# jwliao1209/DiffMusic

Measured on AMD Instinct MI355X. Metric: denoising steps/sec (10 s clip, 200-step DPS), higher is better.
Workload: dtype f16; 1 GPU; MusicLDM + DPS music_inpainting, 10 s @16 kHz, 200-step schedule, batch 8 per GPU (BASELINE.json configs[1]); global_batch=8, clips_per_gpu=8, lanes=1, parallelism=clip-sharded x1 (RCCL world size 1, no per-step collective), finite=True, nan_steps=0, settle_steps=10, cached_reference_transform=True, launched_by=single process

## Files before the change

diffmusic_amd/_ctypes_ops.py:

```python
import ctypes as C

import torch

from . import _lib


def _stream():
    return C.c_void_p(torch.cuda.current_stream().cuda_stream)


def _p(t):
    return C.c_void_p(t.data_ptr()) if t is not None else C.c_void_p(0)


def abi_version():
    return _lib.lib().dmx_abi_version()


def sched_pred_x0(x, eps, alpha_t, *, ptype=0, clip_r=0.0):
    x0 = torch.empty_like(x)
    if ptype == 0 and clip_r == 0.0:
        _lib.check(_lib.lib().dmx_sched_pred_x0(_p(x), _p(eps), _p(x0), x.numel(), alpha_t, _stream()), "pred_x0")
    else:
        _lib.check(_lib.lib().dmx_sched_pred_x0_ex(_p(x), _p(eps), _p(x0), x.numel(), alpha_t, ptype, clip_r, _stream()), "pred_x0_ex")
# ... 461 lines not shown
    return mean, logvar, x


def grad_normalize_(dwav, target):
    inv_scale = torch.empty(dwav.shape[0], dtype=torch.float32, device=dwav.device)
    _lib.check(_lib.lib().dmx_grad_normalize(_p(dwav), _p(inv_scale), dwav.shape[0], dwav.shape[1], target, _stream()), "grad_normalize")
    return inv_scale


def hifigan_fwd(model, mel, ws):
    lib = _lib.lib()
    B, T, _ = mel.shape
    wav = torch.empty(B, lib.dmx_hifigan_out_len(model, T), dtype=torch.float32, device=mel.device)
    _lib.check(lib.dmx_hifigan_fwd(model, _p(mel), _p(wav), B, T, _p(ws), ws.numel(), _stream()), "hifigan_fwd")
    return wav


def hifigan_fwd_dead(model, mel, s0, s1, ws):
    B, T, _ = mel.shape
    lib = _lib.lib()
    wav = torch.empty(B, lib.dmx_hifigan_out_len(model, T), dtype=torch.float32, device=mel.device)
    _lib.check(lib.dmx_hifigan_fwd_dead(model, _p(mel), _p(wav), B, T, int(s0), int(s1), _p(ws), ws.numel(), _stream()), "hifigan_fwd_dead")
    return wav


def hifigan_dead_plan(model, stages):
    n = int(stages)
    arr = [(C.c_int * n)() for _ in range(4)]
    if _lib.lib().dmx_hifigan_dead_plan(model, *arr, n) < 0:
        _lib.check(-1, "hifigan_dead_plan")
    return [int(a[s]) for s in range(n) for a in arr]


def hifigan_bwd(model, dwav, frames, model_in_dim):
    dmel = torch.empty(dwav.shape[0], frames, model_in_dim, dtype=_lib.act_dtype(), device=dwav.device)
    _lib.check(_lib.lib().dmx_hifigan_bwd(model, _p(dwav), _p(dmel), _stream()), "hifigan_bwd")
    return dmel


def htsat_fwd(model, mel, keep_state, ws):
    lib = _lib.lib()
    B, frames, _ = mel.shape
    tokens, channels = C.c_int(), C.c_int()
    _lib.check(lib.dmx_htsat_feature_dims(model, C.byref(tokens), C.byref(channels)), "htsat dims")
    feat = torch.empty(B, tokens.value, channels.value, dtype=torch.float32, device=mel.device)
    _lib.check(lib.dmx_htsat_fwd(model, _p(mel), B, frames, _p(feat), int(keep_state), _p(ws), ws.numel(), _stream()), "htsat_fwd")
    return feat


def htsat_bwd(model, dfeat, scale, frames, bins):
    dmel = torch.empty(dfeat.shape[0], frames, bins, dtype=torch.float32, device=dfeat.device)
    _lib.check(_lib.lib().dmx_htsat_bwd(model, _p(dfeat), _p(scale), _p(dmel), _stream()), "htsat_bwd")
    return dmel


def gram_fwd(feat):
    B, T, Cc = feat.shape
    g = torch.empty(B, Cc, Cc, dtype=torch.float32, device=feat.device)
    _lib.check(_lib.lib().dmx_gram_fwd(_p(feat), _p(g), B, T, Cc, _stream()), "gram_fwd")
    return g


def gram_bwd(feat, dgram):
    B, T, Cc = feat.shape
    d = torch.empty_like(feat)
    _lib.check(_lib.lib().dmx_gram_bwd(_p(feat), _p(dgram), _p(d), B, T, Cc, _stream()), "gram_bwd")
# ... 2 lines not shown
```

diffmusic_amd/_lib.py:

```python
import ctypes as C
import os

_HERE = os.path.dirname(os.path.abspath(__file__))
LIB_PATH = os.environ.get("DMX_LIB_PATH") or os.path.join(_HERE, "lib", "libdiffmusic_hip.so")
MAX_STAGES = 8


class HifiGanConfig(C.Structure):
    _fields_ = [("model_in_dim", C.c_int), ("upsample_initial_channel", C.c_int), ("num_upsamples", C.c_int),
                ("upsample_rates", C.c_int * MAX_STAGES), ("upsample_kernel_sizes", C.c_int * MAX_STAGES),
                ("num_kernels", C.c_int), ("resblock_kernel_sizes", C.c_int * MAX_STAGES),
                ("num_dilations", C.c_int), ("resblock_dilation_sizes", C.c_int * (MAX_STAGES * MAX_STAGES)),
                ("leaky_relu_slope", C.c_float)]


class VaeConfig(C.Structure):
    _fields_ = [("latent_channels", C.c_int), ("out_channels", C.c_int), ("num_blocks", C.c_int),
                ("block_out_channels", C.c_int * MAX_STAGES), ("layers_per_block", C.c_int),
                ("norm_num_groups", C.c_int), ("eps", C.c_float)]


class UNetConfig(C.Structure):
    _fields_ = [("in_channels", C.c_int), ("out_channels", C.c_int), ("num_blocks", C.c_int),
                ("block_out_channels", C.c_int * MAX_STAGES), ("layers_per_block", C.c_int),
# ... 26 lines not shown
                ("XB", C.c_void_p), ("B2", C.c_void_p), ("ldxb", C.c_int), ("ldb2", C.c_int),
                ("colsum", C.c_void_p), ("ln_eps", C.c_float), ("rowstats_in", C.c_void_p), ("rowstats_out", C.c_void_p), ("nslots", C.c_int),
                ("gn_part", C.c_void_p), ("gnb_x", C.c_void_p), ("gnb_scale", C.c_void_p), ("gnb_shift", C.c_void_p),
                ("gnb_ldx", C.c_int), ("gnb_silu", C.c_int), ("gnb_stats", C.c_void_p), ("gnb_cpg", C.c_int)]


EPI_BIAS, EPI_ROWBIAS, EPI_RESID, EPI_ACCUM, EPI_MASK, EPI_LRELU2, EPI_TANH, EPI_F32OUT, EPI_NO_C, EPI_RESID_INV, EPI_MASKBITS, EPI_BITS2, EPI_SOFTBWD = \
    1, 2, 4, 8, 16, 32, 64, 128, 256, 512, 1024, 2048, 4096
EPI_GEGLU, EPI_LNFOLD, EPI_ROWSTATS, EPI_GNSTATS, EPI_GNBWD = 8192, 16384, 32768, 65536, 131072

_SIGS = {
    "dmx_abi_version": (C.c_int, []),
    "dmx_act_dtype": (C.c_int, []),
    "dmx_last_error": (C.c_char_p, []),
    "dmx_hifigan_create": (C.c_void_p, [C.POINTER(HifiGanConfig)]),
    "dmx_vae_decoder_create": (C.c_void_p, [C.POINTER(VaeConfig)]),
    "dmx_unet_create": (C.c_void_p, [C.POINTER(UNetConfig)]),
    "dmx_model_destroy": (None, [C.c_void_p]),
    "dmx_model_num_params": (C.c_int, [C.c_void_p]),
    "dmx_model_param_name": (C.c_char_p, [C.c_void_p, C.c_int]),
    "dmx_model_param_numel": (C.c_size_t, [C.c_void_p, C.c_int]),
    "dmx_model_param_ndim": (C.c_int, [C.c_void_p, C.c_int]),
    "dmx_model_param_dim": (C.c_int, [C.c_void_p, C.c_int, C.c_int]),
    "dmx_model_load_param": (C.c_int, [C.c_void_p, C.c_char_p, C.c_void_p, C.c_size_t]),
    "dmx_model_finalize": (C.c_int, [C.c_void_p, C.c_void_p]),
    "dmx_hifigan_out_len": (C.c_int, [C.c_void_p, C.c_int]),
    "dmx_hifigan_workspace_bytes": (C.c_size_t, [C.c_void_p, C.c_int, C.c_int]),
    "dmx_hifigan_fwd": (C.c_int, [C.c_void_p, C.c_void_p, C.c_void_p, C.c_int, C.c_int, C.c_void_p, C.c_size_t, C.c_void_p]),
    "dmx_hifigan_bwd": (C.c_int, [C.c_void_p, C.c_void_p, C.c_void_p, C.c_void_p]),
    "dmx_hifigan_fwd_dead": (C.c_int, [C.c_void_p, C.c_void_p, C.c_void_p, C.c_int, C.c_int, C.c_int, C.c_int, C.c_void_p, C.c_size_t,
                                       C.c_void_p]),
    "dmx_hifigan_dead_plan": (C.c_int, [C.c_void_p, C.POINTER(C.c_int), C.POINTER(C.c_int), C.POINTER(C.c_int), C.POINTER(C.c_int), C.c_int]),
    "dmx_conv_dead_rows": (C.c_int, [C.c_int] * 9 + [C.POINTER(C.c_int), C.POINTER(C.c_int)]),
    "dmx_vae_workspace_bytes": (C.c_size_t, [C.c_void_p, C.c_int, C.c_int, C.c_int]),
    "dmx_vae_decode_fwd": (C.c_int, [C.c_void_p, C.c_void_p, C.c_float, C.c_void_p, C.c_void_p, C.c_int, C.c_int, C.c_int,
                                     C.c_int, C.c_void_p, C.c_size_t, C.c_void_p]),
    "dmx_vae_decode_bwd": (C.c_int, [C.c_void_p, C.c_void_p, C.c_float, C.c_void_p, C.c_void_p]),
    "dmx_vae_encoder_create": (C.c_void_p, [C.POINTER(VaeConfig)]),
    "dmx_vae_encoder_workspace_bytes": (C.c_size_t, [C.c_void_p, C.c_int, C.c_int, C.c_int]),
    "dmx_vae_encode_fwd": (C.c_int, [C.c_void_p, C.c_void_p, C.c_float, C.c_void_p, C.c_int, C.c_int, C.c_int, C.c_void_p, C.c_size_t,
                                     C.c_void_p]),
    "dmx_latent_init": (C.c_int, [C.c_void_p] * 6 + [C.c_int] * 3 + [C.c_float] * 3 + [C.c_void_p]),
    "dmx_conv2d_raw": (C.c_int, [C.c_void_p] * 4 + [C.c_int] * 9 + [C.c_void_p]),
    "dmx_unet_workspace_bytes": (C.c_size_t, [C.c_void_p, C.c_int, C.c_int, C.c_int]),
    "dmx_unet_fwd": (C.c_int, [C.c_void_p, C.c_void_p, C.c_void_p, C.c_void_p, C.c_void_p, C.c_int, C.c_int, C.c_int,
                               C.c_void_p, C.c_size_t, C.c_void_p]),
    "dmx_unet_fwd_ctx": (C.c_int, [C.c_void_p] * 5 + [C.c_int, C.c_void_p, C.c_int, C.c_void_p, C.c_void_p, C.c_int, C.c_int, C.c_int,
                                   C.c_void_p, C.c_size_t, C.c_void_p]),
    "dmx_unet_workspace_bytes_ctx": (C.c_size_t, [C.c_void_p, C.c_int, C.c_int, C.c_int, C.c_int, C.c_int]),
    "dmx_htsat_create": (C.c_void_p, [C.POINTER(HtsatConfig)]),
    "dmx_htsat_feature_dims": (C.c_int, [C.c_void_p, C.POINTER(C.c_int), C.POINTER(C.c_int)]),
    "dmx_htsat_workspace_bytes": (C.c_size_t, [C.c_void_p, C.c_int, C.c_int]),
    "dmx_htsat_fwd": (C.c_int, [C.c_void_p, C.c_void_p, C.c_int, C.c_int, C.c_void_p, C.c_int, C.c_void_p, C.c_size_t, C.c_void_p]),
    "dmx_htsat_bwd": (C.c_int, [C.c_void_p, C.c_void_p, C.c_void_p, C.c_void_p, C.c_void_p]),
    "dmx_htsat_tape_raw": (C.c_size_t, [C.c_void_p, C.c_int, C.c_int, C.c_int, C.c_void_p, C.c_size_t, C.c_void_p]),
    "dmx_gram_fwd": (C.c_int, [C.c_void_p, C.c_void_p, C.c_int, C.c_int, C.c_int, C.c_void_p]),
    "dmx_gram_bwd": (C.c_int, [C.c_void_p, C.c_void_p, C.c_void_p, C.c_int, C.c_int, C.c_int, C.c_void_p]),
    "dmx_gemm_raw": (C.c_int, [C.c_void_p, C.c_size_t, C.c_void_p]),
    "dmx_prof_begin": (None, []),
    "dmx_prof_end": (C.c_int, [C.POINTER(C.c_double), C.POINTER(C.c_double)]),
    "dmx_flash_attn_raw": (C.c_int, [C.c_void_p, C.c_void_p, C.c_void_p, C.c_void_p, C.c_void_p] + [C.c_int] * 6 + [C.c_float, C.c_void_p]),
    "dmx_flash_attn_ld_raw": (C.c_int, [C.c_void_p] * 5 + [C.c_int] * 8 + [C.c_float, C.POINTER(C.c_int), C.c_void_p]),
    "dmx_softmax_raw": (C.c_int, [C.c_void_p] * 3 + [C.c_longlong, C.c_int, C.c_longlong, C.c_longlong, C.c_int, C.c_void_p]),
    "dmx_softmax_act_raw": (C.c_int, [C.c_void_p] * 3 + [C.c_longlong, C.c_int, C.c_longlong, C.c_int, C.c_void_p]),
    "dmx_transpose_raw": (C.c_int, [C.c_void_p, C.c_void_p, C.c_int, C.c_int, C.c_longlong, C.c_longlong, C.c_int, C.c_int] + [C.c_longlong] * 4
                          + [C.c_void_p]),
# ... 58 lines not shown
                                     C.c_void_p]),
    "dmx_audio_tf_wgrad_segments": (C.c_int, [C.c_int]),
    "dmx_audio_tf_wgrad": (C.c_int, [C.c_void_p, C.c_void_p, C.c_longlong, C.c_void_p, C.c_longlong, C.c_void_p, C.c_int, C.c_int, C.c_void_p]),
    "dmx_audio_eq_update": (C.c_int, [C.c_void_p, C.c_int] + [C.c_void_p] * 3 + [C.c_int, C.c_int] + [C.c_double] * 4 + [C.c_int, C.c_void_p]),
    "dmx_audio_melscale": (C.c_int, [C.c_void_p, C.c_void_p, C.c_void_p, C.c_int, C.c_int, C.c_float, C.c_float, C.c_void_p]),
    "dmx_mask_apply": (C.c_int, [C.c_void_p, C.c_longlong, C.c_void_p, C.c_void_p, C.c_longlong, C.c_int, C.c_int, C.c_int, C.c_void_p]),
    "dmx_l2_loss": (C.c_int, [C.c_void_p, C.c_longlong, C.c_void_p, C.c_void_p, C.c_void_p, C.c_int, C.c_longlong, C.c_float, C.c_void_p]),
    "dmx_track_stitch_fwd": (C.c_int, [C.c_void_p, C.c_longlong, C.c_void_p, C.POINTER(C.c_int)] + [C.c_int] * 4 + [C.c_void_p]),
    "dmx_track_stitch_bwd": (C.c_int, [C.c_void_p, C.c_void_p, C.c_longlong, C.POINTER(C.c_int)] + [C.c_int] * 5 + [C.c_void_p]),
    "dmx_stem_mix_fwd": (C.c_int, [C.c_void_p, C.c_longlong, C.c_void_p, C.POINTER(C.c_float)] + [C.c_int] * 3 + [C.c_void_p]),
    "dmx_stem_mix_bwd": (C.c_int, [C.c_void_p, C.c_void_p, C.c_longlong, C.POINTER(C.c_float)] + [C.c_int] * 4 + [C.c_void_p]),
    "dmx_stem_project": (C.c_int, [C.c_void_p, C.c_longlong, C.c_void_p, C.c_void_p, C.POINTER(C.c_float), C.c_int, C.c_int, C.c_void_p]),
    "dmx_grad_normalize": (C.c_int, [C.c_void_p, C.c_void_p, C.c_int, C.c_longlong, C.c_float, C.c_void_p]),
    "dmx_fir_fwd": (C.c_int, [C.c_void_p, C.c_longlong, C.c_void_p, C.c_void_p, C.c_longlong] + [C.c_int] * 7 + [C.c_void_p]),
    "dmx_fir_bwd": (C.c_int, [C.c_void_p, C.c_longlong, C.c_void_p, C.c_void_p, C.c_void_p, C.c_longlong] + [C.c_int] * 7 + [C.c_void_p]),
    "dmx_fir_clip_fwd": (C.c_int, [C.c_void_p, C.c_longlong, C.c_void_p, C.c_void_p, C.c_longlong] + [C.c_int] * 4 + [C.c_void_p]),
    "dmx_fir_clip_bwd": (C.c_int, [C.c_void_p, C.c_longlong, C.c_void_p, C.c_void_p, C.c_void_p, C.c_longlong] + [C.c_int] * 4 + [C.c_void_p]),
    "dmx_fir_wgrad_workspace_floats": (C.c_size_t, [C.c_int, C.c_int, C.c_int]),
    "dmx_fir_wgrad": (C.c_int, [C.c_void_p, C.c_longlong, C.c_void_p, C.c_longlong, C.c_void_p, C.c_size_t] + [C.c_int] * 4 + [C.c_void_p]),
    "dmx_ir_update": (C.c_int, [C.c_void_p, C.c_int] + [C.c_void_p] * 4 + [C.c_int, C.c_int] + [C.c_double] * 4 + [C.c_int, C.c_void_p]),
    "dmx_sched_pred_x0": (C.c_int, [C.c_void_p, C.c_void_p, C.c_void_p, C.c_longlong, C.c_float, C.c_void_p]),
    "dmx_sched_pred_x0_ex": (C.c_int, [C.c_void_p, C.c_void_p, C.c_void_p, C.c_longlong, C.c_float, C.c_int, C.c_float, C.c_void_p]),
    "dmx_sched_step_ex": (C.c_int, [C.c_int] + [C.c_void_p] * 9 + [C.c_int, C.c_int] + [C.c_float] * 5 + [C.c_int, C.c_int, C.c_float, C.c_void_p]),
    "dmx_sched_cfg_combine": (C.c_int, [C.c_void_p, C.c_void_p, C.c_longlong, C.c_float, C.c_void_p]),
    "dmx_randn_philox": (C.c_int, [C.c_void_p, C.c_int, C.c_longlong, C.POINTER(C.c_ulonglong), C.c_ulonglong, C.c_void_p]),
    "dmx_sched_step": (C.c_int, [C.c_int] + [C.c_void_p] * 9 + [C.c_int, C.c_int] + [C.c_float] * 5 + [C.c_int, C.c_void_p]),
}

ADDED_IN_V4 = ("dmx_vae_encoder_create", "dmx_vae_encoder_workspace_bytes", "dmx_vae_encode_fwd", "dmx_latent_init",
               "dmx_track_stitch_fwd", "dmx_track_stitch_bwd", "dmx_audio_guidance_fwd_shaped", "dmx_audio_guidance_bwd_shaped",
               "dmx_clip_fwd", "dmx_clip_bwd", "dmx_declip_project", "dmx_hifigan_fwd_dead", "dmx_hifigan_dead_plan", "dmx_conv_dead_rows",
               "dmx_fir_clip_fwd", "dmx_fir_clip_bwd", "dmx_fir_wgrad", "dmx_fir_wgrad_workspace_floats", "dmx_ir_update",
               "dmx_stem_mix_fwd", "dmx_stem_mix_bwd", "dmx_stem_project", "dmx_audio_tf_gain", "dmx_audio_tf_frames",
               "dmx_audio_tf_curve", "dmx_audio_tf_wgrad_segments", "dmx_audio_tf_wgrad", "dmx_audio_eq_update", "dmx_drc_fwd", "dmx_drc_bwd")

_lib = None


def check_symbols(h, path=LIB_PATH):
    for name in ADDED_IN_V4:
        if not hasattr(h, name):
            raise RuntimeError(f"{path} reports ABI version {ABI_VERSION} but does not export `{name}` (a build from before the VAE "
                               "encoder / track-mode / declipping / blind-dereverberation / source-separation / time-frequency-masking / blind-equalisation / de-compression entry points): rebuild it (python -m diffmusic_amd.build --force)")


def lib():
    global _lib
    if _lib is None:
        if not os.path.exists(LIB_PATH):
            raise RuntimeError(f"{LIB_PATH} is missing: build it with `python -m diffmusic_amd.build` "
                               "(the diffmusic_amd hot path has no CPU fallback)")
        h = C.CDLL(LIB_PATH)
        for name, (res, args) in _SIGS.items():
            if not hasattr(h, name):
                continue
            fn = getattr(h, name)
            fn.restype, fn.argtypes = res, args
        if h.dmx_abi_version() != ABI_VERSION:
            raise RuntimeError(f"libdiffmusic_hip.so ABI version {h.dmx_abi_version()} != {ABI_VERSION} expected by this package: rebuild it "
                               "(python -m diffmusic_amd.build --force)")
        check_symbols(h)
        _lib = h
    return _lib


ABI_VERSION = 4


def act_dtype():
    import torch
    return torch.float16 if lib().dmx_act_dtype() == 1 else torch.bfloat16


class DmxError(RuntimeError):
    pass

# ... 6 lines not shown
```

diffmusic_amd/csrc/capi.hip:

```cpp
#include "conv_pair.h"
#include "models.h"

#define M_IMPL(m) ((m) ? (m)->impl : nullptr)
#define ST(s) ((hipStream_t)(s))

extern "C" {

int dmx_abi_version(void) { return DMX_ABI_VERSION; }
int dmx_act_dtype(void) { return DMX_ACT_DTYPE; }

dmx_model* dmx_hifigan_create(const dmx_hifigan_config* cfg) {
  if (!cfg || cfg->num_upsamples > DMX_MAX_STAGES || cfg->num_kernels > DMX_MAX_STAGES || cfg->num_dilations > DMX_MAX_STAGES) {
    dmx_set_error("bad hifigan config");
    return nullptr;
  }
  return new dmx_model{dmx_make_hifigan(cfg)};
}
dmx_model* dmx_vae_decoder_create(const dmx_vae_config* cfg) {
  if (!cfg || cfg->num_blocks > DMX_MAX_STAGES) { dmx_set_error("bad vae config"); return nullptr; }
  Model* m = dmx_make_vae(cfg);
  return m ? new dmx_model{m} : nullptr;
}
dmx_model* dmx_unet_create(const dmx_unet_config* cfg) {
  if (!cfg || cfg->num_blocks > DMX_MAX_STAGES) { dmx_set_error("bad unet config"); return nullptr; }
// ... 16 lines not shown
}
int dmx_model_finalize(dmx_model* m, void* stream) {
  std::string missing;
  if (!m->impl->ps.all_loaded(&missing)) { dmx_set_error("parameter '%s' was never loaded", missing.c_str()); return DMX_ERR_PARAM; }
  const int rc = m->impl->finalize(ST(stream));
  if (rc == DMX_OK) m->impl->finalized = true;
  return rc;
}

static int check(dmx_model* m, int kind) {
  if (!m || !m->impl || m->impl->kind != kind) { dmx_set_error("wrong model handle"); return DMX_ERR_STATE; }
  if (!m->impl->finalized) { dmx_set_error("model not finalized"); return DMX_ERR_STATE; }
  return DMX_OK;
}

int dmx_hifigan_out_len(const dmx_model* m, int frames) { return dmx_hifigan_out_len_impl(m->impl, frames); }
size_t dmx_hifigan_workspace_bytes(dmx_model* m, int batch, int frames) { return dmx_hifigan_ws_impl(m->impl, batch, frames); }
int dmx_hifigan_fwd(dmx_model* m, const uint16_t* mel, float* wav, int batch, int frames, void* ws, size_t ws_bytes, void* stream) {
  int rc = check(m, DMX_MODEL_HIFIGAN);
  if (rc) return rc;
  if (!ws) { dmx_set_error("null workspace"); return DMX_ERR_WORKSPACE; }
  return dmx_hifigan_fwd_impl(m->impl, mel, wav, batch, frames, ws, ws_bytes, ST(stream));
}
int dmx_hifigan_fwd_dead(dmx_model* m, const uint16_t* mel, float* wav, int batch, int frames, int s0, int s1, void* ws, size_t ws_bytes,
                         void* stream) {
  int rc = check(m, DMX_MODEL_HIFIGAN);
  if (rc) return rc;
  if (!ws || !mel || !wav) { dmx_set_error("hifigan_fwd_dead: null buffer"); return DMX_ERR_STATE; }
  return dmx_hifigan_fwd_dead_impl(m->impl, mel, wav, batch, frames, s0, s1, ws, ws_bytes, ST(stream));
}
int dmx_hifigan_dead_plan(dmx_model* m, int* skipped, int* total, int* lo, int* hi, int n) {
  if (!m || !m->impl || m->impl->kind != DMX_MODEL_HIFIGAN) { dmx_set_error("wrong model handle"); return -1; }
  return dmx_hifigan_dead_plan_impl(m->impl, skipped, total, lo, hi, n);
}
int dmx_conv_dead_rows(int k, int dil, int pad, int stride, int transposed, int t_in, int t_out, int a, int b, int* lo, int* hi) {
  if (!lo || !hi) return DMX_ERR_STATE;
  return dmx_conv_dead_rows_impl(k, dil, pad, stride, transposed, t_in, t_out, a, b, lo, hi);
}
int dmx_hifigan_bwd(dmx_model* m, const float* dwav, uint16_t* dmel, void* stream) {
  int rc = check(m, DMX_MODEL_HIFIGAN);
  if (rc) return rc;
  return dmx_hifigan_bwd_impl(m->impl, dwav, dmel, ST(stream));
}

size_t dmx_vae_workspace_bytes(dmx_model* m, int batch, int h, int w) { return dmx_vae_ws_impl(m->impl, batch, h, w); }
int dmx_vae_decode_fwd(dmx_model* m, const float* z, float z_scale, uint16_t* mel, float* mel_f32, int batch, int h, int w,
                       int keep_state, void* ws, size_t ws_bytes, void* stream) {
  int rc = check(m, DMX_MODEL_VAE);
  if (rc) return rc;
  if (!ws) { dmx_set_error("null workspace"); return DMX_ERR_WORKSPACE; }
  return dmx_vae_fwd_impl(m->impl, z, z_scale, mel, mel_f32, batch, h, w, keep_state, ws, ws_bytes, ST(stream));
}
int dmx_vae_decode_bwd(dmx_model* m, const uint16_t* dmel, float z_scale, float* dz, void* stream) {
  int rc = check(m, DMX_MODEL_VAE);
  if (rc) return rc;
  return dmx_vae_bwd_impl(m->impl, dmel, z_scale, dz, ST(stream));
}

dmx_model* dmx_vae_encoder_create(const dmx_vae_config* cfg) {
  if (!cfg || cfg->num_blocks > DMX_MAX_STAGES) { dmx_set_error("bad vae config"); return nullptr; }
  Model* m = dmx_make_vae_encoder(cfg);
  return m ? new dmx_model{m} : nullptr;
}
size_t dmx_vae_encoder_workspace_bytes(dmx_model* m, int batch, int frames, int bins) {
  if (!m || !m->impl || m->impl->kind != DMX_MODEL_VAE_ENC) return 0;
  return dmx_vae_enc_ws_impl(m->impl, batch, frames, bins);
// ... 240 lines not shown
```

diffmusic_amd/csrc/dmx_common.h:

```cpp
#pragma once
#include <hip/hip_runtime.h>
#include <stdint.h>
#include <stddef.h>

typedef uint16_t act_t;

#define DMX_OK 0
#define DMX_ERR_SHAPE (-1)
#define DMX_ERR_WORKSPACE (-2)
#define DMX_ERR_PARAM (-3)
#define DMX_ERR_STATE (-4)
#define DMX_ERR_LAUNCH (-5)

typedef __attribute__((ext_vector_type(4))) float f32x4;
#ifdef DMX_BF16
typedef __bf16 native16_t;
typedef __attribute__((ext_vector_type(8))) __bf16 frag8_t;
#define DMX_MFMA16(a, b, c) __builtin_amdgcn_mfma_f32_16x16x32_bf16(a, b, c, 0, 0, 0)
#define DMX_ACT_DTYPE 0
#else
typedef _Float16 native16_t;
typedef __attribute__((ext_vector_type(8))) _Float16 frag8_t;
#define DMX_MFMA16(a, b, c) __builtin_amdgcn_mfma_f32_16x16x32_f16(a, b, c, 0, 0, 0)
#define DMX_ACT_DTYPE 1
// ... 83 lines not shown
  int M, N, K;
  int ldw;
  int Hi, Wi, Ci, lda;
  int Hq, Wq, sy, sx;
  int ntaps;
  int Ho, Wo, ldc, osy, ooy, osx, oox;
  int ldr, ldx, ldc2;
  int Z, Zi;
  long long sAo, sAi, sWo, sWi, sCo, sCi;
  float alpha, act_slope, mask_slope;
  int flags;
  signed char tdy[DMX_MAX_TAPS], tdx[DMX_MAX_TAPS];
  float resid_inv_slope;
  int tile_cfg;
  int ldrb;
  int ksplit;
  const unsigned char* XB;
  unsigned char* B2;
  int ldxb, ldb2;
  const float* colsum;
  float ln_eps;
  const float* rowstats_in;
  float* rowstats_out;
  int nslots;
  float* gn_part;
  const act_t* gnb_x;
  const float* gnb_scale;
  const float* gnb_shift;
  int gnb_ldx, gnb_silu;
  const float* gnb_stats;
  int gnb_cpg;
};

int dmx_gemm_launch(const GemmDesc& d, hipStream_t stream, int* gn_rows = nullptr);
void dmx_gemm_set_splitk_workspace(float* ws, size_t bytes);
void dmx_gemm_release_splitk_workspace(const float* ws);
int dmx_gemm_launch_ln(int cfg, const GemmDesc& d, hipStream_t stream);
int dmx_gemm_launch_rowstats(int cfg, const GemmDesc& d, hipStream_t stream);
int dmx_gemm_launch_gnstats(int cfg, const GemmDesc& d, hipStream_t stream, int* gn_rows);
bool dmx_prof_is_active();
```

diffmusic_amd/csrc/gemm_conv.hip:

```cpp
#include "gemm_tile.h"

namespace {
template <int BM, int BN, int WM, int WN, int NSTAGE>
int launch_glds(const GemmDesc& d, hipStream_t stream) {
  if (d.flags & EPI_SOFTBWD) {
    if constexpr (BM == 256 && BN == 256) return launch_glds_t<BM, BN, WM, WN, NSTAGE, 2>(d, stream);
    else return DMX_ERR_SHAPE;
  }
  if (d.flags & EPI_GEGLU) return launch_glds_t<BM, BN, WM, WN, NSTAGE, 3>(d, stream);
  return (d.flags & (EPI_MASKBITS | EPI_BITS2)) ? launch_glds_t<BM, BN, WM, WN, NSTAGE, 1>(d, stream)
                                                : launch_glds_t<BM, BN, WM, WN, NSTAGE, 0>(d, stream);
}

template <int BM, int BN, int WM, int WN>
int launch_cfg(const GemmDesc& d, hipStream_t stream) {
  if (d.flags & EPI_SOFTBWD) return DMX_ERR_SHAPE;
  if (d.flags & EPI_GEGLU) {
    if constexpr ((BN / WN) % 32 == 0) return launch_cfg_t<BM, BN, WM, WN, 3>(d, stream);
    else return DMX_ERR_SHAPE;
  }
  return (d.flags & (EPI_MASKBITS | EPI_BITS2)) ? launch_cfg_t<BM, BN, WM, WN, 1>(d, stream) : launch_cfg_t<BM, BN, WM, WN, 0>(d, stream);
}

}

#include <vector>
#include <cstdio>
#include <cstdlib>
#include <cmath>
namespace {
struct ProfRec { hipEvent_t a, b; double flops, bytes; int M, N, K, Z, taps, flags, cfg; };
int g_last_cfg = 0;
bool g_prof = false;
std::vector<ProfRec> g_prof_recs;
struct TileEntry { int M, N, K, Z, cfg; };
static const TileEntry g_tile_table[] = {
#include "tile_table.inc"
    {0, 0, 0, 0, 0}};

bool glds_ok(const GemmDesc& d) {
  const long long imgs = d.Hq * d.Wq > 0 ? (d.M + (long long)d.Hq * d.Wq - 1) / ((long long)d.Hq * d.Wq) : 1;
  const long long in_elems = (d.Hi > 1 || d.ntaps > 1 ? imgs * d.Hi * d.Wi : (long long)d.M) * d.lda;
  static const bool strided_ok = getenv("DMX_NO_GLDS_STRIDED") == nullptr;
  return in_elems < (1ll << 29) && (long long)d.M * d.lda < (1ll << 29) && ((long long)d.N + 512) * d.ldw < (1ll << 29) &&
         (d.sy == 1 || strided_ok);
}
int launch_by_cfg(int cfg, const GemmDesc& d, hipStream_t stream, int* gn_rows = nullptr) {
  g_last_cfg = cfg;
  if (d.flags & EPI_LNFOLD) return dmx_gemm_launch_ln(cfg, d, stream);
  if (d.flags & EPI_ROWSTATS) return dmx_gemm_launch_rowstats(cfg, d, stream);
  if (d.flags & (EPI_GNSTATS | EPI_GNBWD)) return dmx_gemm_launch_gnstats(cfg, d, stream, gn_rows);
  switch (cfg) {
    case 1: return launch_glds<256, 256, 2, 4, 2>(d, stream);
    case 2: return launch_glds<256, 128, 4, 2, 3>(d, stream);
    case 7: return launch_glds<320, 256, 2, 4, 2>(d, stream);
    case 8: return launch_glds<192, 256, 2, 4, 2>(d, stream);
    case 9: return launch_glds<320, 128, 4, 2, 2>(d, stream);
    case 10: return launch_glds<192, 128, 4, 2, 3>(d, stream);
    case 11: return launch_glds<128, 128, 2, 2, 2>(d, stream);
    case 12: return launch_glds<64, 64, 2, 2, 4>(d, stream);
    case 13: return launch_glds<128, 64, 2, 2, 3>(d, stream);
    case 14: return launch_glds<64, 128, 2, 2, 3>(d, stream);
    case 15: return launch_glds<64, 64, 2, 2, 8>(d, stream);
    case 16: return launch_glds<64, 128, 2, 2, 6>(d, stream);
    case 17: return launch_glds<128, 64, 2, 2, 6>(d, stream);
    case 18: return launch_glds<128, 128, 2, 2, 4>(d, stream);
    case 19: return launch_glds<512, 128, 4, 2, 2>(d, stream);
    case 3: return launch_cfg<128, 128, 2, 2>(d, stream);
    case 4: return launch_cfg<128, 64, 2, 2>(d, stream);
    case 5: return launch_cfg<128, 32, 4, 1>(d, stream);
    default: return launch_cfg<64, 64, 2, 2>(d, stream);
  }
}
int launch_dispatch(const GemmDesc& d, hipStream_t stream, int* gn_rows) {
  const bool gl = glds_ok(d);
  if (d.flags & EPI_SOFTBWD) return gl ? launch_by_cfg(1, d, stream, gn_rows) : DMX_ERR_SHAPE;
  if (d.tile_cfg >= 1 && d.tile_cfg <= 19 && ((d.tile_cfg > 2 && d.tile_cfg < 7) || gl)) return launch_by_cfg(d.tile_cfg, d, stream, gn_rows);
  {
    static int ovN[8], ovC[8], nov = -1;
    if (nov < 0) {
      nov = 0;
      if (const char* e = getenv("DMX_CFG_OVERRIDE")) {
        while (*e && nov < 8) {
          int n = 0, c = 0;
          if (sscanf(e, "%d:%d", &n, &c) == 2) { ovN[nov] = n; ovC[nov] = c; ++nov; }
          while (*e && *e != ',') ++e;
          if (*e == ',') ++e;
        }
      }
    }
    if (gl && d.M >= 40000)
      for (int i = 0; i < nov; ++i) if (ovN[i] == d.N) return launch_by_cfg(ovC[i], d, stream, gn_rows);
  }
  for (const TileEntry* e = g_tile_table; e->cfg; ++e)
    if (e->M == d.M && e->N == d.N && e->K == d.K && e->Z == d.Z) {
      const int c = e->cfg % 100;
      if ((c > 2 && c < 7) || gl) return launch_by_cfg(c, d, stream, gn_rows);
    }
  if (gl && d.M >= 2048 && d.N % 128 == 0) {
    auto cost = [&](int bm, int bn, int slots, double eff) {
      const double blocks = (double)cdiv(d.M, bm) * cdiv(d.N, bn) * d.Z;
      const double rounds = ceil(blocks / slots);
      return rounds * (bm / 128.0) * (bn / 128.0) * (slots / 256.0) / eff;
    };
    struct Cand { int cfg, bm, bn, slots; double eff; };
    static const Cand cands[] = {{1, 256, 256, 256, 0.95}, {7, 320, 256, 256, 0.93}, {8, 192, 256, 256, 0.88},
                                 {2, 256, 128, 256, 0.70}, {9, 320, 128, 256, 0.70}, {10, 192, 128, 256, 0.66},
                                 {19, 512, 128, 256, 0.75},
                                 {3, 128, 128, 512, 0.66}};
    int best = 0;
    double bc = 1e30;
    for (const Cand& c : cands) {
      if (c.bn == 256 && d.N % 256) continue;
      const double v = cost(c.bm, c.bn, c.slots, c.eff);
      if (v < bc) { bc = v; best = c.cfg; }
    }
    if (best && best != 3) return launch_by_cfg(best, d, stream, gn_rows);
  }
  if (d.N > 32 && (long long)cdiv(d.M, 128) * cdiv(d.N, 128) * d.Z < 200) {
    if (gl && d.K >= 512 && d.Z == 1) return launch_by_cfg(d.N % 128 == 0 && d.M >= 4000 ? 14 : 12, d, stream, gn_rows);
    return launch_by_cfg(6, d, stream, gn_rows);
  }
  if (d.N > 64) return launch_by_cfg(3, d, stream, gn_rows);
  if (d.N > 32) return launch_by_cfg(4, d, stream, gn_rows);
  return launch_by_cfg(5, d, stream, gn_rows);
}
}

bool dmx_prof_is_active() { return g_prof; }

extern "C" void dmx_prof_begin(void) {
  for (auto& r : g_prof_recs) { (void)hipEventDestroy(r.a); (void)hipEventDestroy(r.b); }
  g_prof_recs.clear();
  g_prof = true;
}
static double g_dma_ms = 0.0, g_dma_fl = 0.0, g_dma_by = 0.0;
static int g_dma_n = 0;
#ifdef DMX_GEMM_STAMPS
extern "C" int dmx_gemm_stamps_read(unsigned long long* host) {
  return hipMemcpyFromSymbol(host, HIP_SYMBOL(g_gemm_stamps), sizeof(unsigned long long) * 8192 * 6) == hipSuccess ? 0 : -1;
}
#endif

extern "C" int dmx_prof_dominant(double* ms, double* flops, double* bytes) {
  if (ms) *ms = g_dma_ms;
  if (flops) *flops = g_dma_fl;
  if (bytes) *bytes = g_dma_by;
  return g_dma_n;
}
extern "C" int dmx_prof_end(double* total_ms, double* total_flops) {
  g_prof = false;
  g_dma_ms = g_dma_fl = g_dma_by = 0.0; g_dma_n = 0;
  (void)hipDeviceSynchronize();
  double ms = 0.0, fl = 0.0;
  FILE* csv = getenv("DMX_PROF_CSV") ? fopen(getenv("DMX_PROF_CSV"), "w") : nullptr;
  if (csv) fprintf(csv, "M,N,K,Z,taps,flags,cfg,ms,tflops\n");
  for (auto& r : g_prof_recs) {
    float t = 0.f;
    if (hipEventElapsedTime(&t, r.a, r.b) == hipSuccess) ms += t;
    if (csv) fprintf(csv, "%d,%d,%d,%d,%d,%d,%d,%.4f,%.1f\n", r.M, r.N, r.K, r.Z, r.taps, r.flags, r.cfg, t, t > 0 ? r.flops / t / 1e9 : 0.0);
    const bool dma = r.cfg == 1 || r.cfg == 2 || (r.cfg >= 7 && r.cfg <= 10) || r.cfg == 19;
    if (dma) { g_dma_ms += t; g_dma_fl += r.flops; g_dma_by += r.bytes; ++g_dma_n; }
    fl += r.flops;
    (void)hipEventDestroy(r.a); (void)hipEventDestroy(r.b);
  }
  if (csv) fclose(csv);
  const int n = (int)g_prof_recs.size();
  g_prof_recs.clear();
  if (total_ms) *total_ms = ms;
  if (total_flops) *total_flops = fl;
  return n;
}

namespace {
float* g_splitk_ws = nullptr;
size_t g_splitk_bytes = 0;

__global__ void splitk_epilogue_kernel(const GemmDesc p, const float* __restrict__ ws, int ksplit) {
  const long long q = (long long)blockIdx.x * blockDim.x + threadIdx.x;
  const int nq = p.N >> 2;
  if (q >= (long long)p.M * nq) return;
  const int m = (int)(q / nq), n = (int)(q - (long long)m * nq) * 4;
  const long long mn = (long long)p.M * p.N;
  float4 v = *reinterpret_cast<const float4*>(ws + (long long)m * p.N + n);
  for (int s = 1; s < ksplit; ++s) {
    const float4 w = *reinterpret_cast<const float4*>(ws + s * mn + (long long)m * p.N + n);
    v.x += w.x; v.y += w.y; v.z += w.z; v.w += w.w;
  }
  float a[4] = {v.x, v.y, v.z, v.w};
  const int flags = p.flags;
  const long long row = m;
  if (flags & EPI_MASK) {
    const uint2 xr = *reinterpret_cast<const uint2*>(p.X + row * p.ldx + n);
    const float x[4] = {alo(xr.x), ahi(xr.x), alo(xr.y), ahi(xr.y)};
// ... 60 lines not shown
  g.flags = EPI_F32OUT;
  g.C = g_splitk_ws; g.C2 = nullptr; g.ldc = d.N; g.alpha = 1.f;
  g.bias = nullptr; g.rowbias = nullptr; g.R = nullptr; g.X = nullptr;
  g.Ho = d.Hq; g.Wo = d.Wq;
  g.tile_cfg = 0;
  int rc = launch_by_cfg(tile, g, stream);
  if (rc != DMX_OK) return rc;
  const long long nthr = (long long)d.M * (d.N >> 2);
  hipLaunchKernelGGL(splitk_epilogue_kernel, dim3((unsigned)((nthr + 255) / 256)), dim3(256), 0, stream, d, g_splitk_ws, ks);
  g_last_cfg = 100 * ks + tile;
  return hipGetLastError() == hipSuccess ? DMX_OK : DMX_ERR_LAUNCH;
}
}

void dmx_gemm_set_splitk_workspace(float* ws, size_t bytes) { g_splitk_ws = ws; g_splitk_bytes = bytes; }
void dmx_gemm_release_splitk_workspace(const float* ws) { if (g_splitk_ws == ws) { g_splitk_ws = nullptr; g_splitk_bytes = 0; } }

int dmx_prof_open(hipStream_t st) {
  if (!g_prof) return -1;
  ProfRec r;
  memset(&r, 0, sizeof(r));
  (void)hipEventCreate(&r.a); (void)hipEventCreate(&r.b);
  (void)hipEventRecord(r.a, st);
  g_prof_recs.push_back(r);
  return (int)g_prof_recs.size() - 1;
}
void dmx_prof_close(int rec, hipStream_t st, double flops, double bytes, int M, int N, int K, int taps, int flags, int cfg) {
  if (rec < 0 || rec >= (int)g_prof_recs.size()) return;
  ProfRec& r = g_prof_recs[rec];
  (void)hipEventRecord(r.b, st);
  r.flops = flops; r.bytes = bytes; r.M = M; r.N = N; r.K = K; r.Z = 1; r.taps = taps; r.flags = flags; r.cfg = cfg;
}

int dmx_gemm_launch(const GemmDesc& d, hipStream_t stream, int* gn_rows) {
  if (gn_rows) *gn_rows = 0;
  if (d.M <= 0 || d.N <= 0 || d.K <= 0) return DMX_ERR_SHAPE;
  if ((d.Ci & 7) || (d.N & 3) || (d.K & 7) || (d.lda & 7) || (d.ldw & 7) || (d.ldc & 3)) return DMX_ERR_SHAPE;
  if (d.ntaps < 1 || d.ntaps > DMX_MAX_TAPS || d.K != d.ntaps * d.Ci) return DMX_ERR_SHAPE;
  if (d.Z < 1 || d.Zi < 1) return DMX_ERR_SHAPE;
  if ((d.flags & EPI_LRELU2) && !(d.act_slope >= 0.f && d.act_slope <= 1.f)) return DMX_ERR_SHAPE;
  if ((d.flags & EPI_RESID_INV) && !(d.resid_inv_slope >= 1.f)) return DMX_ERR_SHAPE;
  if (d.flags & EPI_SOFTBWD) {
    if ((d.flags & ~(EPI_SOFTBWD)) || ((d.N | d.ldc | d.ldx) & 7) || !d.X || !d.rowbias || d.Zi != 1 || d.ntaps != 1) return DMX_ERR_SHAPE;
    if (!(d.osy == 1 && d.osx == 1 && d.ooy == 0 && d.oox == 0 && d.Ho == d.Hq && d.Wo == d.Wq)) return DMX_ERR_SHAPE;
  }
  if (d.flags & EPI_GEGLU) {
    if ((d.flags & ~(EPI_GEGLU | EPI_BIAS | EPI_LNFOLD)) || (d.N & 31) || (d.ldc & 7) || d.ldc < d.N / 2 || d.alpha != 1.f) return DMX_ERR_SHAPE;
    if ((d.ldr | d.ldx | d.ldc2) & 7) return DMX_ERR_SHAPE;
    if (!(d.osy == 1 && d.osx == 1 && d.ooy == 0 && d.oox == 0 && d.Ho == d.Hq && d.Wo == d.Wq)) return DMX_ERR_SHAPE;
  }
  if (d.flags & (EPI_MASKBITS | EPI_BITS2)) {
    if ((d.flags & EPI_F32OUT) || ((d.N | d.ldc | d.ldr | d.ldx | d.ldc2) & 7) || d.Z != 1) return DMX_ERR_SHAPE;
    if ((d.flags & EPI_MASKBITS) && (!d.XB || d.ldxb * 8 < d.N)) return DMX_ERR_SHAPE;
    if ((d.flags & EPI_BITS2) && (!d.B2 || d.ldb2 * 8 < d.N)) return DMX_ERR_SHAPE;
  }
  if ((d.flags & EPI_LNFOLD) && (d.flags & EPI_BIAS)) {
    GemmDesc q = d;
    q.flags &= ~EPI_BIAS;
    return dmx_gemm_launch(q, stream, gn_rows);
  }
  if (d.flags & EPI_LNFOLD) {
    if (d.ntaps != 1 || d.K != d.Ci || !d.colsum || !d.rowstats_in || d.nslots < 1 || d.Z != 1 ||
        (d.flags & (EPI_F32OUT | EPI_MASK | EPI_MASKBITS | EPI_BITS2 | EPI_SOFTBWD | EPI_ACCUM | EPI_TANH | EPI_LRELU2 | EPI_ROWSTATS)))
      return DMX_ERR_SHAPE;
  }
  if (d.flags & EPI_ROWSTATS) {
// ... 40 lines not shown
```

diffmusic_amd/csrc/gemm_epilogue.h:

```cpp
#pragma once
#include "dmx_common.h"
#include <type_traits>

namespace {

template <int I, int N, typename F>
__device__ __forceinline__ void static_for(F&& f) {
  if constexpr (I < N) {
    f(std::integral_constant<int, I>{});
    static_for<I + 1, N>(f);
  }
}


template <int FM, int FN>
__device__ __forceinline__ void gemm_epilogue(const GemmDesc& p, f32x4 (&acc)[FM][FN], int m0, int n0, int lr, int lq,
                                              long long coff, int HqWq) {
  const int flags = p.flags;
#pragma unroll
  for (int i = 0; i < FM; ++i) {
    const int m = m0 + i * 16 + lr;
    if (m >= p.M) continue;
    const int b = m / HqWq, rem = m - b * HqWq;
    const int qy = rem / p.Wq, qx = rem - qy * p.Wq;
// ... 42 lines not shown
        act_t* cp = reinterpret_cast<act_t*>(p.C) + coff + orow * p.ldc + n;
        if (flags & EPI_ACCUM) {
          const uint2 o = *reinterpret_cast<const uint2*>(cp);
          v[0] += alo(o.x); v[1] += ahi(o.x); v[2] += alo(o.y); v[3] += ahi(o.y);
        }
        if (flags & EPI_TANH) { v[0] = tanhf(v[0]); v[1] = tanhf(v[1]); v[2] = tanhf(v[2]); v[3] = tanhf(v[3]); }
        if (!(flags & EPI_NO_C)) *reinterpret_cast<uint2*>(cp) = make_uint2(pack2a(v[0], v[1]), pack2a(v[2], v[3]));
      }
      if (flags & EPI_LRELU2) {
        const float s = p.act_slope;
        const float a0 = v[0] > 0.f ? v[0] : v[0] * s, a1 = v[1] > 0.f ? v[1] : v[1] * s;
        const float a2 = v[2] > 0.f ? v[2] : v[2] * s, a3 = v[3] > 0.f ? v[3] : v[3] * s;
        *reinterpret_cast<uint2*>(p.C2 + coff + orow * p.ldc2 + n) = make_uint2(pack2a(a0, a1), pack2a(a2, a3));
      }
    }
  }
}

__device__ __forceinline__ unsigned dmx_pos8(const uint4& v) {
  auto pos = [](uint32_t u) -> uint32_t { return (((u & 0x7fff7fffu) + 0x7fff7fffu) & ~u) & 0x80008000u; };
  const uint32_t w = (pos(v.x) >> 15) | (pos(v.y) >> 13) | (pos(v.z) >> 11) | (pos(v.w) >> 9);
  return (w & 0x55u) | ((w >> 15) & 0xaau);
}

#ifndef DMX_GNB_HB
#define DMX_GNB_HB 4
#endif
#ifndef DMX_EPI_IB
#define DMX_EPI_IB 4
#endif
template <int FM>
struct EpiChunk { static constexpr int IB = (FM % DMX_EPI_IB == 0) ? DMX_EPI_IB : (FM % 4 == 0) ? 4 : (FM % 3 == 0) ? 3 : (FM % 2 == 0) ? 2 : 1; static constexpr int CH = IB * 16; };

template <int FM, int FN, int EM>
__device__ __forceinline__ void gemm_epilogue_lds_impl(const GemmDesc& p, f32x4 (&acc)[FM][FN], int m0, int n0, int lane,
                                                       long long coff, int HqWq, char* wl, int mlimit,
                                                       const uint2 (&rpre)[FM * FN], const bool use_rpre) {
  constexpr bool BITS = EM == 1;
  constexpr bool SOFT = EM == 2;
  constexpr bool GEGLU = EM == 3;
  constexpr bool ROWS = EM == 4;
  static_assert(!ROWS || FN == 2 || FN == 4, "row statistics come in slots of 32 columns");
  constexpr bool GNS = EM == 5;
  constexpr bool GNB = EM == 6;
  static_assert(!GEGLU || FN % 2 == 0, "GEGLU pairs accumulator fragments");
  constexpr int CH = EpiChunk<FM>::CH;
  constexpr int IB = EpiChunk<FM>::IB;
  constexpr int TNB = FN * 32;
  constexpr int PITCH = TNB + 16;
  constexpr int CPR = TNB / 16;
  constexpr int RPI = 64 / CPR;
  constexpr int NIT = CH / RPI;
  static_assert(CH % RPI == 0, "chunk rows must be a multiple of the rows per wave-instruction");
  const int lr = lane & 15, lq = lane >> 4;
  const int rr = lane / CPR, cch = lane - rr * CPR;
  int* tab = reinterpret_cast<int*>(wl + CH * PITCH);
  const int flags = p.flags;
  const int ncol = n0 + cch * 8;
  const bool col_ok = ncol < p.N;
  const int mend = p.M < mlimit ? p.M : mlimit;
  const bool ident = p.osy == 1 && p.osx == 1 && p.ooy == 0 && p.oox == 0 && p.Ho == p.Hq && p.Wo == p.Wq;
#define DMX_LDS_SYNC() asm volatile("s_waitcnt lgkmcnt(0)" ::: "memory")
  float4 bcol[FN];
#pragma unroll
  for (int j = 0; j < FN; ++j) {
    const int n = n0 + j * 16 + lq * 4;
    bcol[j] = ((flags & EPI_BIAS) && n < p.N) ? *reinterpret_cast<const float4*>(p.bias + n) : make_float4(0.f, 0.f, 0.f, 0.f);
  }
  float gs[4] = {0.f, 0.f, 0.f, 0.f};
  constexpr int GN_SLOT = 64;
  static_assert(!(GNS || GNB) || (CH == GN_SLOT && FN == 4), "GroupNorm statistics: 64-row chunks of 64-column wave tiles only (one summation order)");
  const int gn_b0 = (GNS || GNB) ? m0 / HqWq : 0;
  static_for<0, FM / IB>([&](auto H) {
    constexpr int h = decltype(H)::value;
    int orows[NIT];
    if (ident) {
#pragma unroll
      for (int it = 0; it < NIT; ++it) {
        const int m = m0 + h * CH + it * RPI + rr;
        orows[it] = m < mend ? m : -1;
      }
    } else {
      if (lane < CH) {
        const int m = m0 + h * CH + lane;
        int orow = -1;
        if (m < mend) {
          const int b = m / HqWq, rem = m - b * HqWq;
          const int qy = rem / p.Wq, qx = rem - qy * p.Wq;
          orow = (b * p.Ho + (qy * p.osy + p.ooy)) * p.Wo + (qx * p.osx + p.oox);
        }
        tab[lane] = orow;
      }
      DMX_LDS_SYNC();
#pragma unroll
      for (int it = 0; it < NIT; ++it) orows[it] = tab[it * RPI + rr];
      DMX_LDS_SYNC();
    }
    auto stage_in = [&](const act_t* G, int ld, auto&& f) {
      {
        uint4 v[NIT];
#pragma unroll
        for (int it = 0; it < NIT; ++it) {
          const bool ok = orows[it] >= 0 && col_ok;
          const long long off = ok ? (long long)orows[it] * ld + ncol : 0ll;
          v[it] = *reinterpret_cast<const uint4*>(G + coff + off);
          if (!ok) v[it] = make_uint4(0, 0, 0, 0);
        }
#pragma unroll
        for (int it = 0; it < NIT; ++it) *reinterpret_cast<uint4*>(wl + (it * RPI + rr) * PITCH + cch * 16) = v[it];
      }
      DMX_LDS_SYNC();
#pragma unroll
      for (int ii = 0; ii < IB; ++ii)
#pragma unroll
        for (int j = 0; j < FN; ++j) {
          const uint2 q = *reinterpret_cast<const uint2*>(wl + (ii * 16 + lr) * PITCH + (j * 16 + lq * 4) * 2);
          f(acc[h * IB + ii][j], alo(q.x), ahi(q.x), alo(q.y), ahi(q.y));
        }
      DMX_LDS_SYNC();
    };
    auto stage_out = [&](act_t* G, int ld, auto&& f) {
      constexpr int JS = GEGLU ? 2 : 1;
      static_for<0, IB>([&](auto II) {
        static_for<0, FN / JS>([&](auto JJ) {
          constexpr int ii = decltype(II)::value, j = decltype(JJ)::value * JS;
          float o[4];
          f(acc[h * IB + ii][j], o);
          *reinterpret_cast<uint2*>(wl + (ii * 16 + lr) * PITCH + ((j / JS) * 16 + lq * 4) * 2) = make_uint2(pack2a(o[0], o[1]), pack2a(o[2], o[3]));
        });
      });
      DMX_LDS_SYNC();
      constexpr int HN = NIT > 4 ? NIT / 2 : NIT;
#pragma unroll
      for (int g0 = 0; g0 < NIT; g0 += HN) {
      uint4 v[HN];
#pragma unroll
// ... 175 lines not shown
          if (flags & EPI_ROWBIAS) {
            const float4 bb = *reinterpret_cast<const float4*>(p.rowbias + (long long)bimg * (p.ldrb ? p.ldrb : p.N) + n);
            a[0] += bb.x; a[1] += bb.y; a[2] += bb.z; a[3] += bb.w;
          }
        }
      }
    }
    if constexpr (GEGLU) {
#pragma unroll
      for (int ii = 0; ii < IB; ++ii)
#pragma unroll
        for (int j = 0; j < FN; j += 2) {
          f32x4& a = acc[h * IB + ii][j];
          const f32x4& g = acc[h * IB + ii][j + 1];
#pragma unroll
          for (int e = 0; e < 4; ++e) a[e] *= 0.5f * g[e] * erfcf(g[e] * -0.70710678118654752f);
        }
    }
    if ((flags & EPI_RESID) && use_rpre) {
      const float is = (flags & EPI_RESID_INV) ? p.resid_inv_slope : 1.f;
#pragma unroll
      for (int ii = 0; ii < IB; ++ii)
#pragma unroll
        for (int j = 0; j < FN; ++j) {
          const uint2 q = rpre[(h * IB + ii) * FN + j];
          const float x0 = alo(q.x), x1 = ahi(q.x), x2 = alo(q.y), x3 = ahi(q.y);
          f32x4& a = acc[h * IB + ii][j];
          a[0] += fminf(x0, x0 * is); a[1] += fminf(x1, x1 * is); a[2] += fminf(x2, x2 * is); a[3] += fminf(x3, x3 * is);
        }
    } else if (flags & EPI_RESID) {
      const float is = (flags & EPI_RESID_INV) ? p.resid_inv_slope : 1.f;
      stage_in(p.R, p.ldr, [&](f32x4& a, float x0, float x1, float x2, float x3) {
        a[0] += fminf(x0, x0 * is); a[1] += fminf(x1, x1 * is); a[2] += fminf(x2, x2 * is); a[3] += fminf(x3, x3 * is);
      });
    }
    if (p.alpha != 1.f) {
      const float al = p.alpha;
#pragma unroll
      for (int ii = 0; ii < IB; ++ii)
#pragma unroll
        for (int j = 0; j < FN; ++j) { f32x4& a = acc[h * IB + ii][j]; a[0] *= al; a[1] *= al; a[2] *= al; a[3] *= al; }
    }
    if (flags & EPI_ACCUM)
      stage_in(reinterpret_cast<const act_t*>(p.C), p.ldc, [&](f32x4& a, float x0, float x1, float x2, float x3) { a[0] += x0; a[1] += x1; a[2] += x2; a[3] += x3; });
    if (flags & EPI_TANH) {
#pragma unroll
      for (int ii = 0; ii < IB; ++ii)
#pragma unroll
        for (int j = 0; j < FN; ++j) { f32x4& a = acc[h * IB + ii][j]; a[0] = tanhf(a[0]); a[1] = tanhf(a[1]); a[2] = tanhf(a[2]); a[3] = tanhf(a[3]); }
    }
    if constexpr (ROWS) {
      if (flags & EPI_ROWSTATS) {
        float2* rso = reinterpret_cast<float2*>(p.rowstats_out);
        const int ns = p.nslots;
#pragma unroll
        for (int ii = 0; ii < IB; ++ii) {
          const int m = m0 + h * CH + ii * 16 + lr;
#pragma unroll
          for (int sl = 0; sl < FN / 2; ++sl) {
            float sv = 0.f, qv = 0.f;
#pragma unroll
            for (int jj = 0; jj < 2; ++jj) {
              const int j = sl * 2 + jj;
              const f32x4& a = acc[h * IB + ii][j];
              if (n0 + j * 16 + lq * 4 < p.N) {
                sv += (a[0] + a[1]) + (a[2] + a[3]);
                qv += (a[0] * a[0] + a[1] * a[1]) + (a[2] * a[2] + a[3] * a[3]);
// ... 12 lines not shown
      stage_out(reinterpret_cast<act_t*>(p.C), p.ldc, [&](const f32x4& a, float (&o)[4]) { o[0] = a[0]; o[1] = a[1]; o[2] = a[2]; o[3] = a[3]; });
      if constexpr (BITS) { if (bits2 && !(flags & EPI_LRELU2)) emit_bits(); }
      if constexpr (GNS) { if (flags & EPI_GNSTATS) emit_gn(); }
      if constexpr (GNB) { if (flags & EPI_GNBWD) emit_gnb(); }
      if constexpr (GNS || GNB) {
        if ((flags & (EPI_GNSTATS | EPI_GNBWD)) && m0 + h * CH < mend) {
#pragma unroll
          for (int o = CPR; o < 64; o <<= 1) {
#pragma unroll
            for (int k = 0; k < 4; ++k) gs[k] += __shfl_xor(gs[k], o, 64);
          }
          if (rr == 0 && col_ok) {
            const int nq = p.N >> 2, slots = (HqWq + GN_SLOT - 1) / GN_SLOT + 1;
            float* dst = p.gn_part + (((long long)gn_b0 * slots + (m0 + h * CH - gn_b0 * HqWq) / GN_SLOT) * nq + (ncol >> 2)) * 2;
            *reinterpret_cast<float4*>(dst) = make_float4(gs[0], gs[1], gs[2], gs[3]);
          }
        }
        gs[0] = gs[1] = gs[2] = gs[3] = 0.f;
      }
      DMX_LDS_SYNC();
    }
    if (flags & EPI_LRELU2) {
      const float sl = p.act_slope;
      stage_out(p.C2, p.ldc2, [&](const f32x4& a, float (&o)[4]) {
        o[0] = fmaxf(a[0], a[0] * sl); o[1] = fmaxf(a[1], a[1] * sl); o[2] = fmaxf(a[2], a[2] * sl); o[3] = fmaxf(a[3], a[3] * sl);
      });
      if constexpr (BITS) { if (bits2) emit_bits(); }
      DMX_LDS_SYNC();
    }
  });
#undef DMX_LDS_SYNC
}

template <int FM, int FN, int EM>
__device__ __forceinline__ void gemm_epilogue_lds(const GemmDesc& p, f32x4 (&acc)[FM][FN], int m0, int n0, int lane,
                                                  long long coff, int HqWq, char* wl, int mlimit = 0x7fffffff) {
  const uint2 none[FM * FN] = {};
  gemm_epilogue_lds_impl<FM, FN, EM>(p, acc, m0, n0, lane, coff, HqWq, wl, mlimit, none, false);
}

}
```

diffmusic_amd/csrc/gemm_tile.h:

```cpp
#pragma once
#include "dmx_common.h"
#include <type_traits>
#include <cstdlib>

#include "gemm_epilogue.h"
#include "conv_pair.h"

namespace {

constexpr int BK = 64;
constexpr int DMX_DEF_BIG = 0;

template <int BM, int BN, int NT>
__device__ __forceinline__ void ln_prologue(const GemmDesc& p, int m0, int n0, float2* s_ln, float* s_cs) {
  constexpr int TPR = NT / BM >= 4 ? 4 : (NT / BM >= 2 ? 2 : 1);
  const int tid = threadIdx.x, ns = p.nslots;
  const int r = tid / TPR, sub = tid - r * TPR;
  const float inv_c = 1.f / (float)p.K;
  if (r < BM) {
    const int m = m0 + r;
    const bool row_ok = m < p.M;
    const float2* rs = reinterpret_cast<const float2*>(p.rowstats_in) + (long long)(row_ok ? m : 0) * ns;
    float si = 0.f, qi = 0.f;
    for (int t0 = 0; t0 < ns; t0 += TPR * 8) {
// ... 176 lines not shown
      for (int i = 0; i < FM; ++i) af[i] = *reinterpret_cast<const frag8_t*>(sa + i * 16 * 128 + sw);
#pragma unroll
      for (int j = 0; j < FN; ++j) wf[j] = *reinterpret_cast<const frag8_t*>(sb + j * 16 * 128 + sw);
#pragma unroll
      for (int i = 0; i < FM; ++i)
#pragma unroll
        for (int j = 0; j < FN; ++j)
          acc[i][j] = DMX_MFMA16(wf[j], af[i], acc[i][j]);
    }
    if (ks + 1 < nk) store_tile(cur ^ 1);
    __syncthreads();
  }
  if constexpr (LNF) ln_apply<FM, FN, BN>(acc, s_ln, s_cs, wm * TM, wn * TN, lr, lq);

  if ((p.flags & EPI_F32OUT) || ((p.N | p.ldc | p.ldr | p.ldx | p.ldc2) & 7)) {
    gemm_epilogue<FM, FN>(p, acc, m0t + wm * TM, tn * BN + wn * TN, lr, lq, coff, HqWq);
  } else {
    constexpr int EPI_CH = EpiChunk<FM>::CH;
    constexpr int EPI_WAVE_BYTES = EPI_CH * (FN * 32 + 16) + EPI_CH * 12;
    static_assert(EPI_WAVE_BYTES * WM * WN <= 2 * (BM + BN) * 128, "epilogue staging does not fit the stage buffers");
    gemm_epilogue_lds<FM, FN, EM>(p, acc, m0t + wm * TM, tn * BN + wn * TN, lane, coff, HqWq, smem + wave * EPI_WAVE_BYTES, mlim);
  }
}

constexpr unsigned OOB = 0x80000000u;

#ifdef DMX_GEMM_STAMPS
__device__ unsigned long long g_gemm_stamps[8192 * 6];
#define DMX_GSTAMP(i) do { gstamp_v[i] = wall_clock64(); } while (0)
#else
#define DMX_GSTAMP(i) do { } while (0)
#endif

template <int BM, int BN, int WM, int WN, int NSTAGE, int EM, bool LNF = false>
__device__ __forceinline__ void glds_tile(const GemmDesc& p, char* smem, const int m0, const int tn, const int mlim) {
  constexpr int NW = WM * WN;
  constexpr int TM = BM / WM, TN = BN / WN;
  constexpr int FM = TM / 16, FN = TN / 16;
  constexpr int A_ISS = BM / 8 / NW, B_ISS = BN / 8 / NW;
  constexpr int A_BYTES = BM * 128, B_BYTES = BN * 128, STAGE = A_BYTES + B_BYTES;
  static_assert(A_ISS >= 1 && B_ISS >= 1, "tile too small");

  constexpr int PER = A_ISS + B_ISS;
  constexpr int KEEP = (NSTAGE - 2) * PER;

  const int tid = threadIdx.x;
  const int wave = __builtin_amdgcn_readfirstlane(tid >> 6), lane = tid & 63;
#ifdef DMX_GEMM_STAMPS
  unsigned long long gstamp_v[5] = {0, 0, 0, 0, 0};
#endif
  DMX_GSTAMP(0);
  const int z = blockIdx.y;
  const int zo = z / p.Zi, zi = z - zo * p.Zi;
  const act_t* Ab = p.A + zo * p.sAo + zi * p.sAi;
  const act_t* Wb = p.W + zo * p.sWo + zi * p.sWi;
  const int nsplit = p.ksplit > 1 ? p.ksplit : 1, sp = blockIdx.z;
  const long long coff = zo * p.sCo + zi * p.sCi + (nsplit > 1 ? (long long)sp * p.M * p.N : 0ll);
  const __amdgpu_buffer_rsrc_t rsA = __builtin_amdgcn_make_buffer_rsrc(const_cast<act_t*>(Ab), 0, OOB, 0x00020000);
  const __amdgpu_buffer_rsrc_t rsW = __builtin_amdgcn_make_buffer_rsrc(const_cast<act_t*>(Wb), 0, (unsigned)p.N * (unsigned)p.ldw * 2u, 0x00020000);

  int tapreg = 0;
#pragma unroll
  for (int j = 0; j < DMX_MAX_TAPS; ++j)
    if (lane == j) tapreg = (int)(unsigned char)p.tdy[j] | ((int)(unsigned char)p.tdx[j] << 8);

  const int lrow = lane >> 3, cc = (lane & 7) ^ lrow;
  const int cpt = p.Ci >> 3;
  const int HqWq = p.Hq * p.Wq;
  const unsigned lda2 = (unsigned)p.lda * 2u;
  unsigned a_lin[A_ISS], a_mask2[(A_ISS + 1) / 2];
  {
    int r_iy[A_ISS], r_ix[A_ISS];
    unsigned r_mask[A_ISS];
#pragma unroll
    for (int i = 0; i < A_ISS; ++i) {
      const int m = m0 + (i * NW + wave) * 8 + lrow;
      r_mask[i] = 0u; a_lin[i] = 0u;
      r_iy[i] = -(1 << 20); r_ix[i] = 0;
      if (m < mlim) {
        int b = 0, qy = 0, qx = m;
        if (!(p.Hq == 1 && p.Wq >= p.M)) {
          b = m / HqWq; const int rem = m - b * HqWq;
          qy = rem / p.Wq; qx = rem - qy * p.Wq;
        }
        r_iy[i] = qy * p.sy; r_ix[i] = qx * p.sx;
        a_lin[i] = (unsigned)b * (unsigned)(p.Hi * p.Wi) * lda2 + (unsigned)(r_iy[i] * p.Wi + r_ix[i]) * lda2 + ((unsigned)cc << 4);
      }
    }
    for (int t = 0; t < p.ntaps; ++t) {
      const int tv = __builtin_amdgcn_readlane(tapreg, t);
      const int dy = (int)(signed char)(tv & 0xff), dx = (int)(signed char)((tv >> 8) & 0xff);
#pragma unroll
      for (int i = 0; i < A_ISS; ++i)
        if ((unsigned)(r_iy[i] + dy) < (unsigned)p.Hi && (unsigned)(r_ix[i] + dx) < (unsigned)p.Wi) r_mask[i] |= 1u << t;
    }
#pragma unroll
    for (int i = 0; i < (A_ISS + 1) / 2; ++i) a_mask2[i] = 0u;
#pragma unroll
    for (int i = 0; i < A_ISS; ++i) a_mask2[i >> 1] |= r_mask[i] << ((i & 1) * 16);
  }
  const unsigned ldw2 = (unsigned)p.ldw * 2u;
  const unsigned w_row = (unsigned)(tn * BN + wave * 8 + lrow) * ldw2;
  const unsigned w_step = (unsigned)(NW * 8) * ldw2;

  const int kchunks = p.K >> 3;
  const bool tap_inner = (p.Ci & 63) == 0 || p.ntaps == 1;
  const int cgroups = (p.Ci + 63) >> 6;
  const int nk_all = (p.K + BK - 1) / BK;
  const int ks_per = (nk_all + nsplit - 1) / nsplit;
  const int ks0 = sp * ks_per, ks1 = ks0 + ks_per < nk_all ? ks0 + ks_per : nk_all;
  int i_cg = ks0 / p.ntaps, i_tp = ks0 - i_cg * p.ntaps;
  bool q_kval = false;
  int q_tp = 0;
  unsigned q_adel = 0, q_wdel = 0;
  char* q_base = nullptr;
  auto issue_begin = [&](int ksl, int stage) {
    q_base = smem + stage * STAGE;
    if (tap_inner) {
      const int tp = __builtin_amdgcn_readfirstlane(i_tp), cgi = __builtin_amdgcn_readfirstlane(i_cg);
      q_kval = cgi < cgroups && ksl + ks0 < ks1 && cgi * 8 + cc < cpt;
      const int tv = __builtin_amdgcn_readlane(tapreg, tp);
      const int dy = (int)(signed char)(tv & 0xff), dx = (int)(signed char)((tv >> 8) & 0xff);
      q_tp = tp;
      q_adel = (unsigned)((dy * p.Wi + dx) * (int)lda2) + ((unsigned)cgi << 7);
      q_wdel = (unsigned)(tp * cpt + cgi * 8 + cc) << 4;
      if (++i_tp == p.ntaps) { i_tp = 0; ++i_cg; }
    } else {
// ... 138 lines not shown
        });
      } else {
        static_for<0, NS>([&](auto ST) {
          constexpr int st = decltype(ST)::value;
          read_step(ST);
          wait_step(ST);
          mfma_step(ST);
          if constexpr (st < SPREAD) {
            static_for<st * PER / SPREAD, (st + 1) * PER / SPREAD>(issue_one);
            __builtin_amdgcn_sched_barrier(0);
          }
        });
      }
      asm volatile("s_waitcnt vmcnt(%0)\n\ts_waitcnt lgkmcnt(0)" ::"n"(KEEP) : "memory");
      __builtin_amdgcn_s_barrier();
      cur = cur + 1 == NSTAGE ? 0 : cur + 1;
      nxt = nxt + 1 == NSTAGE ? 0 : nxt + 1;
    }
    if constexpr (LAG) {
      __builtin_amdgcn_sched_barrier(0);
      if (nk > 0) static_for<LOWN, NS>(mfma_step);
    }
  };
  if constexpr (STAGGER) {
    if (wave >= NW / 2) kloop(std::true_type{}); else kloop(std::false_type{});
  } else {
    kloop(std::false_type{});
  }
#undef DMX_DSR
  asm volatile("s_waitcnt vmcnt(0)" ::: "memory");
  __builtin_amdgcn_s_barrier();
  DMX_GSTAMP(2);
  if constexpr (LNF) ln_apply<FM, FN, BN>(acc, s_ln, s_cs, wm * TM, wn * TN, lr, lq);
  if ((p.flags & EPI_F32OUT) || ((p.N | p.ldc | p.ldr | p.ldx | p.ldc2) & 7)) {
    gemm_epilogue<FM, FN>(p, acc, m0 + wm * TM, tn * BN + wn * TN, lr, lq, coff, HqWq);
  } else {
    constexpr int EPI_CH = EpiChunk<FM>::CH;
    constexpr int EPI_WAVE_BYTES = EPI_CH * (FN * 32 + 16) + EPI_CH * 12;
    static_assert(EPI_WAVE_BYTES * WM * WN <= 2 * (BM + BN) * 128, "epilogue staging does not fit the stage buffers");
    gemm_epilogue_lds<FM, FN, EM>(p, acc, m0 + wm * TM, tn * BN + wn * TN, lane, coff, HqWq, smem + wave * EPI_WAVE_BYTES, mlim);
  }
#ifdef DMX_GEMM_STAMPS
  DMX_GSTAMP(3);
  asm volatile("s_waitcnt vmcnt(0)" ::: "memory");
  DMX_GSTAMP(4);
  {
    const int wg = blockIdx.x + gridDim.x * (blockIdx.y + gridDim.y * blockIdx.z);
    if (tid == NW * 64 - 64 && wg < 8192) {
      unsigned hw, xcc;
      asm volatile("s_getreg_b32 %0, hwreg(HW_REG_HW_ID)" : "=s"(hw));
      asm volatile("s_getreg_b32 %0, hwreg(HW_REG_XCC_ID)" : "=s"(xcc));
#pragma unroll
      for (int i = 0; i < 5; ++i) g_gemm_stamps[wg * 6 + i] = gstamp_v[i];
      g_gemm_stamps[wg * 6 + 5] = ((unsigned long long)(xcc & 0xf) << 32) | hw;
    }
  }
#endif
}

__device__ __forceinline__ int xcd_remap(int bid) {
  const int nwg = gridDim.x, q = nwg >> 3, r = nwg & 7, xcd = bid & 7, loc = bid >> 3;
  return (xcd < r ? xcd * (q + 1) : r * (q + 1) + (xcd - r) * q) + loc;
}

template <int BM, int BN, int WM, int WN, int NSTAGE, int EM, bool LNF = false>
__global__ __launch_bounds__(WM* WN * 64) void gemm_glds_kernel(const GemmDesc p) {
// ... 70 lines not shown
```

diffmusic_amd/csrc/hifigan.hip:

```cpp
#include "models.h"
#include "conv_pair.h"
#include <cstdlib>

struct SplitKScope {
  explicit SplitKScope(float* ws, size_t bytes, bool on) : on_(on && ws) { if (on_) dmx_gemm_set_splitk_workspace(ws, bytes); }
  ~SplitKScope() { if (on_) dmx_gemm_set_splitk_workspace(nullptr, 0); }
  bool on_;
};

struct Span { int a = 0, b = 0; bool empty() const { return b <= a; } };
static inline Span span_meet(Span x, Span y) { Span r{x.a > y.a ? x.a : y.a, x.b < y.b ? x.b : y.b}; if (r.empty()) r = Span{}; return r; }
static inline long long floor_div(long long a, long long b) { return a >= 0 ? a / b : -((-a + b - 1) / b); }
static inline long long ceil_div(long long a, long long b) { return -floor_div(-a, b); }

int dmx_conv_dead_rows_impl(int k, int dil, int pad, int stride, int transposed, int t_in, int t_out, int a, int b, int* lo, int* hi) {
  *lo = *hi = 0;
  if (k < 1 || dil < 1 || stride < 1 || pad < 0 || t_in < 1 || t_out < 1) return DMX_ERR_SHAPE;
  if (!transposed && stride != 1) return DMX_ERR_SHAPE;
  if (a < 0) a = 0;
  if (b > t_out) b = t_out;
  if (b <= a) return DMX_OK;
  const long long INF = 1ll << 40;
  const long long ea = a == 0 ? -INF : a, eb = b == t_out ? INF : b;
  long long l, h;
  if (!transposed) {
    l = ea - pad + (long long)(k - 1) * dil;
    h = eb - pad;
  } else {
    l = ceil_div(ea + pad, stride);
    h = ceil_div(eb - (k - 1) + pad, stride);
  }
  if (l < 0) l = 0;
  if (h > t_in) h = t_in;
  if (h > l) { *lo = (int)l; *hi = (int)h; }
  return DMX_OK;
}
static Span dead_in(const ConvLayer& L, Span d, int t_in, int t_out) {
  Span r;
  (void)dmx_conv_dead_rows_impl(L.kw, L.dil, L.pad_w, L.stride, L.transposed ? 1 : 0, t_in, t_out, d.a, d.b, &r.a, &r.b);
  return r;
}

struct DeadPlan {
  int B = 0, T = 0, s0 = 0, s1 = 0;
  bool on = false;
  Span wav;
  std::vector<Span> out, xs;
  std::vector<Span> xo, h, x;
  std::vector<int> skipped, total;
};

struct HifiGan : Model {
  dmx_hifigan_config cfg;
  DeadPlan plan;
  bool use_dead = false;
  static constexpr size_t kSplitKBytes = 32u << 20;
  float* splitk_ws = nullptr;
  ConvLayer conv_pre, conv_post;
  std::vector<ConvLayer> ups;
  std::vector<ConvLayer> c1, c2;
  int nk = 0, nd = 0, ns = 0;
  int B = 0, T = 0;
  std::vector<int> Ts;
  act_t* act_pre = nullptr;
  std::vector<act_t*> xs_a;
  std::vector<act_t*> ha, xa;
  std::vector<act_t*> act_out;
  std::vector<unsigned char*> hb, xb;
  std::vector<char> fused;
  float* wav8 = nullptr;
  bool have_tape = false;
  hipStream_t bstream[DMX_MAX_STAGES] = {};
  std::vector<hipEvent_t> events;
  size_t ev_next = 0;
  bool want_multi = true;
  hipEvent_t next_event() { hipEvent_t e = events[ev_next]; ev_next = (ev_next + 1) % events.size(); return e; }
  bool multi() const { return want_multi && !dry && !dmx_prof_is_active() && nk > 1; }
  bool multi_wanted() const { return want_multi && nk > 1; }

  int idx(int s, int k, int d) const { return (s * nk + k) * nd + d; }

  explicit HifiGan(const dmx_hifigan_config& c) : cfg(c) {
    kind = DMX_MODEL_HIFIGAN;
    ns = c.num_upsamples; nk = c.num_kernels; nd = c.num_dilations;
    const int C0 = c.upsample_initial_channel;
    conv_pre = make_conv1d(ps, "conv_pre", c.model_in_dim, C0, 7, 1, 3, true);
    for (int i = 0; i < ns; ++i) {
      const int s = c.upsample_rates[i], k = c.upsample_kernel_sizes[i];
      ups.push_back(make_convT1d(ps, "upsampler." + std::to_string(i), C0 >> i, C0 >> (i + 1), k, s, (k - s) / 2, true));
    }
    int ch = C0;
    for (int i = 0; i < ns; ++i) {
      ch = C0 >> (i + 1);
      for (int j = 0; j < nk; ++j) {
        const int k = c.resblock_kernel_sizes[j];
        const std::string pre = "resblocks." + std::to_string(i * nk + j);
        for (int d = 0; d < nd; ++d) {
          const int dil = c.resblock_dilation_sizes[j * nd + d];
          c1.push_back(make_conv1d(ps, pre + ".convs1." + std::to_string(d), ch, ch, k, dil, (k * dil - dil) / 2, true));
          c2.push_back(make_conv1d(ps, pre + ".convs2." + std::to_string(d), ch, ch, k, 1, (k - 1) / 2, true));
        }
      }
    }
    conv_post = make_conv1d(ps, "conv_post", ch, 1, 7, 1, 3, true);
    want_multi = getenv("DMX_MULTI_STREAM") != nullptr && getenv("DMX_SINGLE_STREAM") == nullptr;
    for (int k = 1; k < nk; ++k) (void)hipStreamCreateWithFlags(&bstream[k], hipStreamNonBlocking);
    events.resize(256);
    for (auto& e : events) (void)hipEventCreateWithFlags(&e, hipEventDisableTiming);
    splitk_ws = (float*)ps.dalloc(kSplitKBytes);
  }
  ~HifiGan() override {
    dmx_gemm_release_splitk_workspace(splitk_ws);
    for (int k = 1; k < nk; ++k) if (bstream[k]) (void)hipStreamDestroy(bstream[k]);
    for (auto& e : events) (void)hipEventDestroy(e);
  }

  int finalize(hipStream_t st) override {
    int rc = pack_layer(ps, conv_pre, st);
    for (auto& l : ups) if (rc == DMX_OK) rc = pack_layer(ps, l, st);
    for (auto& l : c1) if (rc == DMX_OK) rc = pack_layer(ps, l, st);
    for (auto& l : c2) if (rc == DMX_OK) rc = pack_layer(ps, l, st);
    if (rc == DMX_OK) rc = pack_layer(ps, conv_post, st);
    return rc;
  }

  bool step_is_fused(int id, int To) const {
    GemmDesc da, db;
    act_t* dummy = reinterpret_cast<act_t*>(size_t(256));
    unsigned char* dummyb = reinterpret_cast<unsigned char*>(size_t(256));
    Epi ea; ea.flags = EPI_LRELU2 | EPI_NO_C | EPI_BITS2; ea.act_slope = cfg.leaky_relu_slope; ea.B2 = dummyb;
    if (conv_fwd_1d_desc(c1[id], dummy, nullptr, B, To, ea, da) != DMX_OK) return false;
    Epi eb; eb.flags = EPI_RESID | EPI_RESID_INV | EPI_LRELU2 | EPI_NO_C | EPI_ACCUM; eb.R = dummy; eb.C2 = dummy;
    eb.resid_inv_slope = 1.f / cfg.leaky_relu_slope; eb.act_slope = cfg.leaky_relu_slope;
    if (conv_fwd_1d_desc(c2[id], nullptr, dummy, B, To, eb, db) != DMX_OK) return false;
    return dmx_conv_pair_eligible(&da, db);
  }

  void step_slabs(int id, int To, bool bwd, const PairDead& pd, int& skipped, int& total) const {
    GemmDesc da, db;
    act_t* dummy = reinterpret_cast<act_t*>(size_t(256));
    unsigned char* dummyb = reinterpret_cast<unsigned char*>(size_t(256));
    skipped = total = 0;
    if (!bwd) {
      Epi ea; ea.flags = EPI_LRELU2 | EPI_NO_C | EPI_BITS2; ea.act_slope = cfg.leaky_relu_slope; ea.B2 = dummyb;
      Epi eb; eb.flags = EPI_RESID | EPI_RESID_INV; eb.R = dummy; eb.resid_inv_slope = 1.f / cfg.leaky_relu_slope;
      if (conv_fwd_1d_desc(c1[id], dummy, nullptr, B, To, ea, da) != DMX_OK || conv_fwd_1d_desc(c2[id], nullptr, dummy, B, To, eb, db) != DMX_OK) return;
    } else {
      Epi ea; ea.flags = EPI_MASKBITS; ea.mask_slope = cfg.leaky_relu_slope; ea.XB = dummyb;
      Epi eb; eb.flags = EPI_RESID | EPI_MASKBITS; eb.mask_slope = cfg.leaky_relu_slope; eb.R = dummy; eb.XB = dummyb;
      if (conv_bwd_1d_desc(c2[id], dummy, dummy, B, To, ea, da) != DMX_OK || conv_bwd_1d_desc(c1[id], dummy, dummy, B, To, eb, db) != DMX_OK) return;
    }
    dmx_conv_pair_slabs(&da, db, &pd, &skipped, &total);
  }
  bool stage_all_fused(int s, int To) const {
    bool all = nk <= 3;
    for (int k = 0; k < nk; ++k) for (int d = 0; d < nd; ++d) all = all && step_is_fused(idx(s, k, d), To);
    return all;
  }
  PairDead dead_fwd(int id) const {
    const Span w = span_meet(plan.xo[id], plan.h[id]);
    PairDead pd; pd.skip0 = w.a; pd.skip1 = w.b;
    return pd;
  }
  PairDead dead_bwd(int s, int id, int d) const {
    const Span w = d == 0 ? plan.xs[s] : plan.x[id];
    PairDead pd; pd.skip0 = w.a; pd.skip1 = w.b; pd.zero0 = plan.xo[id].a; pd.zero1 = plan.xo[id].b;
    return pd;
  }

  void make_plan(int T_, int s0, int s1) {
    if (plan.B == B && plan.T == T_ && plan.s0 == s0 && plan.s1 == s1 && (int)plan.out.size() == ns) return;
    plan = DeadPlan();
    plan.B = B; plan.T = T_; plan.s0 = s0; plan.s1 = s1;
    plan.out.assign(ns, Span{}); plan.xs.assign(ns, Span{});
    plan.xo.assign(ns * nk * nd, Span{}); plan.h.assign(ns * nk * nd, Span{}); plan.x.assign(ns * nk * nd, Span{});
    plan.skipped.assign(ns, 0); plan.total.assign(ns, 0);
    std::vector<int> len(ns);
    int t = T_;
    for (int i = 0; i < ns; ++i) { t = conv_out_len(ups[i], t); len[i] = t; }
    const int Tout = ns ? len[ns - 1] : T_;
    plan.wav = span_meet(Span{s0, s1}, Span{0, Tout});
    if (plan.wav.empty() || ns == 0) return;
    Span cur = dead_in(conv_post, plan.wav, Tout, Tout);
    for (int s = ns - 1; s >= 0; --s) {
      const int To = len[s], Tin = s ? len[s - 1] : T_;
      plan.out[s] = cur;
      Span xs{0, To};
      for (int k = 0; k < nk; ++k) {
        Span o = cur;
        for (int d = nd - 1; d >= 0; --d) {
          const int id = idx(s, k, d);
          plan.xo[id] = o;
          plan.h[id] = dead_in(c2[id], o, To, To);
          plan.x[id] = span_meet(dead_in(c1[id], plan.h[id], To, To), o);
          o = plan.x[id];
        }
        xs = span_meet(xs, o);
      }
      plan.xs[s] = xs;
      cur = dead_in(ups[s], xs, Tin, To);
    }
    if (multi_wanted()) return;
    int any = 0;
    for (int s = 0; s < ns; ++s) {
      if (!stage_all_fused(s, len[s])) continue;
      for (int k = 0; k < nk; ++k)
        for (int d = 0; d < nd; ++d) {
          const int id = idx(s, k, d);
          int sk, tot;
          step_slabs(id, len[s], false, dead_fwd(id), sk, tot);
          plan.skipped[s] += sk; plan.total[s] += tot;
          step_slabs(id, len[s], true, dead_bwd(s, id, d), sk, tot);
          plan.skipped[s] += sk; plan.total[s] += tot;
        }
      any += plan.skipped[s];
    }
    plan.on = any > 0;
    if (!plan.on) plan.skipped.assign(ns, 0);
  }

  int out_len(int T_) const {
    int t = T_;
    for (int i = 0; i < ns; ++i) t = conv_out_len(ups[i], t);
    return t;
  }

  int forward(const act_t* mel, float* wav, int B_, int T_, void* ws, size_t ws_bytes, hipStream_t st, int s0 = 0, int s1 = 0) {
    if (cfg.model_in_dim & 7) return DMX_ERR_SHAPE;
    dry = (ws == nullptr);
    B = B_;
    if (!dry) {
      use_dead = false;
      if (s1 > s0) { make_plan(T_, s0, s1); use_dead = plan.on; }
    }
    const bool dead = use_dead && !dry;
    SplitKScope sk_scope(splitk_ws, kSplitKBytes, !dry && !multi_wanted());
    arena.reset(ws, dry ? (size_t)-1 : ws_bytes);
    T = T_;
    Ts.assign(ns, 0);
    xs_a.assign(ns, nullptr); act_out.assign(ns, nullptr);
    ha.assign(ns * nk * nd, nullptr); xa.assign(ns * nk * nd, nullptr);
    hb.assign(ns * nk * nd, nullptr); xb.assign(ns * nk * nd, nullptr);
    fused.assign(ns * nk * nd, 0);
    const float slope = cfg.leaky_relu_slope;
    auto bits = [&](size_t rows, int C) { return (unsigned char*)arena.raw(rows * (size_t)(C >> 3)); };
    act_pre = arena.bf((size_t)B * T * conv_pre.Cop);
    {
      Epi e; e.flags = EPI_LRELU2 | EPI_NO_C; e.act_slope = slope; e.C2 = act_pre;
      RUN(conv_fwd_1d(conv_pre, mel, act_pre, B, T, e, st));
    }
    const act_t* cur_act = act_pre;
    int Tin = T;
    for (int s = 0; s < ns; ++s) {
      const ConvLayer& up = ups[s];
      const int To = conv_out_len(up, Tin), C = up.Cop;
      const size_t n = (size_t)B * To * C;
      Ts[s] = To;
      xs_a[s] = arena.bf(n);
      act_out[s] = arena.bf(n);
      unsigned char* xs_b = nullptr;
      for (int k = 0; k < nk; ++k)
        for (int d = 0; d < nd; ++d) {
          const int id = idx(s, k, d);
          fused[id] = step_is_fused(id, To) ? 1 : 0;
          xa[id] = d == 0 ? xs_a[s] : arena.bf(n);
          if (fused[id]) {
// ... 31 lines not shown
              const int idn = idx(s, k, d + 1);
              act_t* xn = xa[idn];
              Epi e; e.flags = EPI_RESID | EPI_RESID_INV | EPI_LRELU2 | EPI_NO_C | EPI_BITS2; e.R = xa[id]; e.resid_inv_slope = 1.f / slope;
              e.act_slope = slope; e.C2 = xn; e.B2 = xb[idn];
              RUN(conv_fwd_1d_desc(c2[id], ha[id], xn, B, To, e, db[k]));
            } else {
              Epi e; e.flags = EPI_RESID | EPI_RESID_INV; e.R = xa[id]; e.resid_inv_slope = 1.f / slope; e.alpha = 1.f / nk;
              if (k > 0) e.flags |= EPI_ACCUM;
              if (k == nk - 1) { e.flags |= EPI_LRELU2 | EPI_NO_C; e.act_slope = next_slope; e.C2 = act_out[s]; }
              RUN(conv_fwd_1d_desc(c2[id], ha[id], sum, B, To, e, db[k]));
            }
            pa[k] = &da[k]; pb[k] = &db[k];
          }
          if (dry) continue;
          for (int k = 0; k < nk; ++k)
            if (!dmx_conv_pair_eligible(&da[k], db[k])) {
              dmx_set_error("hifigan: resblock step %d was planned as fused but the pair kernel refuses it", idx(s, k, d));
              return DMX_ERR_STATE;
            }
          if (d < nd - 1) RUN(dmx_conv_pair_group_launch(nk, pa, pb, st, dead ? pd : nullptr));
          else for (int k = 0; k < nk; ++k) RUN(conv_pair_run(da[k], db[k], st, dead ? &pd[k] : nullptr));
        }
        arena.release(mk);
        cur_act = act_out[s];
        Tin = To;
        continue;
      }
      hipEvent_t fin_prev = nullptr;
      if (mt) {
        hipEvent_t e0 = next_event();
        (void)hipEventRecord(e0, st);
        for (int k = 1; k < nk; ++k) (void)hipStreamWaitEvent(bstream[k], e0, 0);
      }
      for (int k = 0; k < nk; ++k) {
        hipStream_t sk = (mt && k > 0) ? bstream[k] : st;
        for (int d = 0; d < nd; ++d) {
          const int id = idx(s, k, d);
          const bool fz = fused[id] != 0;
          GemmDesc da, db;
          {
            Epi e; e.flags = EPI_LRELU2 | EPI_NO_C; e.act_slope = slope;
            if (fz) { e.flags |= EPI_BITS2; e.B2 = hb[id]; } else e.C2 = ha[id];
            RUN(conv_fwd_1d_desc(c1[id], xa[id], ha[id], B, To, e, da));
          }
          if (d < nd - 1) {
            const int idn = idx(s, k, d + 1);
            act_t* xn = xa[idn];
            Epi e; e.flags = EPI_RESID | EPI_RESID_INV | EPI_LRELU2 | EPI_NO_C; e.R = xa[id]; e.resid_inv_slope = 1.f / slope;
            e.act_slope = slope; e.C2 = xn;
            if (fused[idn]) { e.flags |= EPI_BITS2; e.B2 = xb[idn]; }
            RUN(conv_fwd_1d_desc(c2[id], ha[id], xn, B, To, e, db));
          } else {
            Epi e; e.flags = EPI_RESID | EPI_RESID_INV; e.R = xa[id]; e.resid_inv_slope = 1.f / slope; e.alpha = 1.f / nk;
            if (k > 0) e.flags |= EPI_ACCUM;
            if (k == nk - 1) { e.flags |= EPI_LRELU2 | EPI_NO_C; e.act_slope = next_slope; e.C2 = act_out[s]; }
            RUN(conv_fwd_1d_desc(c2[id], ha[id], sum, B, To, e, db));
          }
          if (!dry && fz && !dmx_conv_pair_eligible(&da, db)) {
            dmx_set_error("hifigan: resblock step %d was planned as fused but the pair kernel refuses it", id);
            return DMX_ERR_STATE;
          }
          if (d == nd - 1 && mt && fin_prev) (void)hipStreamWaitEvent(sk, fin_prev, 0);
          RUN(conv_pair_run(da, db, sk));
          if (d == nd - 1 && mt) { fin_prev = next_event(); (void)hipEventRecord(fin_prev, sk); }
        }
      }
      if (mt && fin_prev) (void)hipStreamWaitEvent(st, fin_prev, 0);
      arena.release(mk);
      cur_act = act_out[s];
      Tin = To;
    }
    const int Tout = Tin;
    wav8 = arena.f32((size_t)B * Tout * 8);
    CHECK_WS("hifigan");
    {
      Epi e; e.flags = EPI_F32OUT | EPI_TANH;
      RUN(conv_fwd_1d(conv_post, cur_act, wav8, B, Tout, e, st));
    }
    if (dead) RUN(dmx_gather_col_f32_dead(wav8, wav, (long long)B * Tout, 8, 0, Tout, plan.wav.a, plan.wav.b, st));
    else RUN(dmx_gather_col_f32(wav8, wav, (long long)B * Tout, 8, 0, st));
    have_tape = true;
    return DMX_OK;
  }

  int backward(const float* dwav, act_t* dmel, hipStream_t st) {
    if (!have_tape && !dry) { dmx_set_error("hifigan backward without forward"); return DMX_ERR_STATE; }
    SplitKScope sk_scope(splitk_ws, kSplitKBytes, !dry && !multi_wanted());
    const float slope = cfg.leaky_relu_slope;
    const int Tout = Ts[ns - 1];
    const size_t mk0 = arena.mark();
    act_t* gz = arena.bf((size_t)B * Tout * 8);
    const int Clast = ups[ns - 1].Cop;
    act_t* g = arena.bf((size_t)B * Tout * Clast);
    CHECK_WS("hifigan");
    const bool dead = use_dead && !dry;
    if (dead) RUN(dmx_tanh_bwd_pad8_dead(dwav, wav8, gz, (long long)B * Tout, Tout, plan.wav.a, plan.wav.b, st));
    else RUN(dmx_tanh_bwd_pad8(dwav, wav8, gz, (long long)B * Tout, st));
    {
      Epi e; e.flags = EPI_MASK; e.X = act_out[ns - 1]; e.mask_slope = 0.01f; e.alpha = 1.f / nk;
      RUN(conv_bwd_1d(conv_post, gz, g, B, Tout, e, st));
    }
    for (int s = ns - 1; s >= 0; --s) {
      const int To = Ts[s], Tin = s == 0 ? T : Ts[s - 1], C = ups[s].Cop;
      const size_t n = (size_t)B * To * C;
      act_t* gxs = arena.bf(n);
      act_t* ghk[DMX_MAX_STAGES];
      act_t* gAB[DMX_MAX_STAGES][2];
      for (int k = 0; k < nk; ++k) { ghk[k] = arena.bf(n); gAB[k][0] = arena.bf(n); gAB[k][1] = arena.bf(n); }
      const int Cin = ups[s].Cip;
      act_t* gprev = arena.bf((size_t)B * Tin * Cin);
      CHECK_WS("hifigan");
      const bool mt = multi();
      hipEvent_t fin_prev = nullptr;
      bool all_fused = nk <= 3;
      for (int k = 0; k < nk; ++k) for (int d = 0; d < nd; ++d) all_fused = all_fused && fused[idx(s, k, d)] != 0;
      if (all_fused && !mt) {
        const act_t* gcs[DMX_MAX_STAGES];
        for (int k = 0; k < nk; ++k) gcs[k] = g;
        if (dead && !plan.xs[s].empty() &&
            hipMemset2DAsync(gxs + (size_t)plan.xs[s].a * C, (size_t)To * C * sizeof(act_t), 0, (size_t)(plan.xs[s].b - plan.xs[s].a) * C * sizeof(act_t),
                             (size_t)B, st) != hipSuccess) {
          dmx_set_error("hifigan: clearing the dead rows of a stage gradient failed");
          return DMX_ERR_LAUNCH;
        }
        for (int d = nd - 1; d >= 0; --d) {
          GemmDesc da[DMX_MAX_STAGES], db[DMX_MAX_STAGES];
          const GemmDesc* pa[DMX_MAX_STAGES]; const GemmDesc* pb[DMX_MAX_STAGES];
          act_t* dsts[DMX_MAX_STAGES];
          PairDead pd[DMX_MAX_STAGES];
          for (int k = 0; k < nk; ++k) {
            const int id = idx(s, k, d);
            if (dead) pd[k] = dead_bwd(s, id, d);
            {
              Epi e; e.mask_slope = slope; e.flags = EPI_MASKBITS; e.XB = hb[id];
              RUN(conv_bwd_1d_desc(c2[id], gcs[k], ghk[k], B, To, e, da[k]));
            }
            Epi e; e.flags = EPI_RESID | EPI_MASKBITS; e.mask_slope = slope; e.R = gcs[k]; e.XB = xb[id];
            if (d == 0) { dsts[k] = gxs; if (k > 0) e.flags |= EPI_ACCUM; }
            else dsts[k] = (gcs[k] == gAB[k][0]) ? gAB[k][1] : gAB[k][0];
            RUN(conv_bwd_1d_desc(c1[id], ghk[k], dsts[k], B, To, e, db[k]));
            pa[k] = &da[k]; pb[k] = &db[k];
          }
          if (!dry) {
            if (d > 0) RUN(dmx_conv_pair_group_launch(nk, pa, pb, st, dead ? pd : nullptr));
            else for (int k = 0; k < nk; ++k) RUN(conv_pair_run(da[k], db[k], st, dead ? &pd[k] : nullptr));
          }
          for (int k = 0; k < nk; ++k) gcs[k] = dsts[k];
        }
      } else {
      if (mt) {
        hipEvent_t e0 = next_event();
        (void)hipEventRecord(e0, st);
        for (int k = 1; k < nk; ++k) (void)hipStreamWaitEvent(bstream[k], e0, 0);
      }
      for (int k = 0; k < nk; ++k) {
        hipStream_t sk = (mt && k > 0) ? bstream[k] : st;
        const act_t* gc = g;
        for (int d = nd - 1; d >= 0; --d) {
          const int id = idx(s, k, d);
          GemmDesc da, db;
          {
            Epi e; e.mask_slope = slope;
            if (fused[id]) { e.flags = EPI_MASKBITS; e.XB = hb[id]; } else { e.flags = EPI_MASK; e.X = ha[id]; }
            RUN(conv_bwd_1d_desc(c2[id], gc, ghk[k], B, To, e, da));
          }
          Epi e; e.flags = EPI_RESID; e.mask_slope = slope; e.R = gc;
          if (fused[id]) { e.flags |= EPI_MASKBITS; e.XB = xb[id]; } else { e.flags |= EPI_MASK; e.X = xa[id]; }
          act_t* dst;
          if (d == 0) {
            dst = gxs;
            if (k > 0) e.flags |= EPI_ACCUM;
            if (mt && fin_prev) (void)hipStreamWaitEvent(sk, fin_prev, 0);
          } else {
            dst = (gc == gAB[k][0]) ? gAB[k][1] : gAB[k][0];
          }
          RUN(conv_bwd_1d_desc(c1[id], ghk[k], dst, B, To, e, db));
          RUN(conv_pair_run(da, db, sk));
          if (d == 0 && mt) { fin_prev = next_event(); (void)hipEventRecord(fin_prev, sk); }
          gc = dst;
        }
      }
      }
      if (mt && fin_prev) (void)hipStreamWaitEvent(st, fin_prev, 0);
      {
        Epi e; e.flags = EPI_MASK; e.mask_slope = slope;
        if (s > 0) { e.X = act_out[s - 1]; e.alpha = 1.f / nk; } else { e.X = act_pre; }
        RUN(conv_bwd_1d(ups[s], gxs, gprev, B, Tin, e, st));
      }
      g = gprev;
    }
    {
      Epi e;
      RUN(conv_bwd_1d(conv_pre, g, dmel, B, T, e, st));
    }
    arena.release(mk0);
    return DMX_OK;
  }
};

Model* dmx_make_hifigan(const dmx_hifigan_config* c) { return new HifiGan(*c); }
int dmx_hifigan_out_len_impl(Model* m, int T) { return static_cast<HifiGan*>(m)->out_len(T); }
int dmx_hifigan_fwd_impl(Model* m, const act_t* mel, float* wav, int B, int T, void* ws, size_t wsb, hipStream_t st) {
  return static_cast<HifiGan*>(m)->forward(mel, wav, B, T, ws, wsb, st);
}
int dmx_hifigan_fwd_dead_impl(Model* m, const act_t* mel, float* wav, int B, int T, int s0, int s1, void* ws, size_t wsb, hipStream_t st) {
  return static_cast<HifiGan*>(m)->forward(mel, wav, B, T, ws, wsb, st, s0, s1);
}
int dmx_hifigan_dead_plan_impl(Model* m, int* skipped, int* total, int* lo, int* hi, int n) {
  HifiGan* h = static_cast<HifiGan*>(m);
  for (int s = 0; s < n && s < h->ns; ++s) {
    const bool have = h->use_dead && s < (int)h->plan.out.size();
    if (skipped) skipped[s] = have ? h->plan.skipped[s] : 0;
    if (total) total[s] = have ? h->plan.total[s] : 0;
    if (lo) lo[s] = have ? h->plan.out[s].a : 0;
    if (hi) hi[s] = have ? h->plan.out[s].b : 0;
  }
  return h->ns;
}
int dmx_hifigan_bwd_impl(Model* m, const float* dwav, act_t* dmel, hipStream_t st) {
  return static_cast<HifiGan*>(m)->backward(dwav, dmel, st);
}
size_t dmx_hifigan_ws_impl(Model* m, int B, int T) {
  HifiGan* h = static_cast<HifiGan*>(m);
  h->arena.peak = 0;
  h->forward(nullptr, nullptr, B, T, nullptr, 0, nullptr);
  h->backward(nullptr, nullptr, nullptr);
  h->have_tape = false;
  h->dry = false;
  return h->arena.peak + 256;
}
```

diffmusic_amd/csrc/models.h:

```cpp
#pragma once
#include "layers.h"
#include "../../include/diffmusic_hip.h"

enum { DMX_MODEL_HIFIGAN = 1, DMX_MODEL_VAE = 2, DMX_MODEL_UNET = 3, DMX_MODEL_HTSAT = 4, DMX_MODEL_VAE_ENC = 5 };

struct Model {
  int kind = 0;
  ParamStore ps;
  Arena arena;
  bool finalized = false;
  bool dry = false;
  virtual ~Model() { ps.free_all(); }
  virtual int finalize(hipStream_t st) = 0;
};
struct dmx_model { Model* impl; };

#define RUN(expr) do { if (!dry) { int rc_ = (expr); if (rc_ != DMX_OK) return rc_; } } while (0)
#define CHECK_WS(name) do { if (arena.overflow) { dmx_set_error(name " workspace too small: need %zu bytes", arena.peak); return DMX_ERR_WORKSPACE; } } while (0)

Model* dmx_make_hifigan(const dmx_hifigan_config* c);
int dmx_hifigan_out_len_impl(Model* m, int T);
int dmx_hifigan_fwd_impl(Model* m, const act_t* mel, float* wav, int B, int T, void* ws, size_t wsb, hipStream_t st);
int dmx_hifigan_bwd_impl(Model* m, const float* dwav, act_t* dmel, hipStream_t st);
int dmx_hifigan_fwd_dead_impl(Model* m, const act_t* mel, float* wav, int B, int T, int s0, int s1, void* ws, size_t wsb, hipStream_t st);
int dmx_hifigan_dead_plan_impl(Model* m, int* skipped, int* total, int* lo, int* hi, int n);
int dmx_conv_dead_rows_impl(int k, int dil, int pad, int stride, int transposed, int t_in, int t_out, int a, int b, int* lo, int* hi);
size_t dmx_hifigan_ws_impl(Model* m, int B, int T);

Model* dmx_make_vae(const dmx_vae_config* c);
size_t dmx_vae_ws_impl(Model* m, int B, int h, int w);
int dmx_vae_fwd_impl(Model* m, const float* z, float zs, act_t* mel, float* mel32, int B, int h, int w, int keep, void* ws, size_t wsb,
                     hipStream_t st);
int dmx_vae_bwd_impl(Model* m, const act_t* dmel, float zs, float* dz, hipStream_t st);
Model* dmx_make_vae_encoder(const dmx_vae_config* c);
size_t dmx_vae_enc_ws_impl(Model* m, int B, int T, int F);
int dmx_vae_enc_fwd_impl(Model* m, const float* mel, float log_floor, float* moments, int B, int T, int F, void* ws, size_t wsb, hipStream_t st);
int dmx_latent_init_impl(const float* moments, float* mean, float* logvar, float* x, const float* eps, const float* noise, int B, int L, int P,
                         float sqrt_abar, float scaling_factor, float sqrt_1m_abar, hipStream_t st);
int dmx_conv2d_raw_impl(const float* w_host, const float* b_host, const act_t* x, act_t* y, int B, int Hi, int Wi, int Ci, int Co, int k,
                        int stride, int pad_lo, int pad_hi, hipStream_t st);
Model* dmx_make_unet(const dmx_unet_config* c);
size_t dmx_unet_ws_impl(Model* m, int B, int h, int w, int n0, int n1);
int dmx_unet_fwd_impl(Model* m, const float* x, const float* t, const float* cls, float* eps, int B, int h, int w, void* ws, size_t wsb,
                      hipStream_t st, const float* c0, int n0, const float* c1, int n1, const float* bias1);

Model* dmx_make_htsat(const dmx_htsat_config* c);
size_t dmx_htsat_ws_impl(Model* m, int B, int frames);
int dmx_htsat_fwd_impl(Model* m, const float* mel, int B, int frames, float* feat, int keep, void* ws, size_t wsb, hipStream_t st);
int dmx_htsat_bwd_impl(Model* m, const float* dfeat, const float* scale, float* dmel, hipStream_t st);
void dmx_htsat_dims_impl(Model* m, int* tokens, int* channels);
size_t dmx_htsat_tape_impl(Model* m, int stage, int block, int which, const act_t** p);
int dmx_gram_fwd_impl(const float* F, float* G, int B, int T, int C, hipStream_t st);
int dmx_gram_bwd_impl(const float* F, const float* dG, float* dF, int B, int T, int C, hipStream_t st);
```

diffmusic_amd/csrc_torch/torch_ops.cpp:

```cpp
#include <ATen/ATen.h>
#include <ATen/hip/impl/HIPGuardImplMasqueradingAsCUDA.h>
#include <ATen/hip/impl/HIPStreamMasqueradingAsCUDA.h>
#include <c10/hip/HIPStream.h>
#include <torch/library.h>

#include "../../include/diffmusic_hip.h"

#pragma weak dmx_vae_encoder_create
#pragma weak dmx_vae_encoder_workspace_bytes
#pragma weak dmx_vae_encode_fwd
#pragma weak dmx_latent_init
#pragma weak dmx_track_stitch_fwd
#pragma weak dmx_track_stitch_bwd
#pragma weak dmx_audio_guidance_fwd_shaped
#pragma weak dmx_audio_guidance_bwd_shaped
#pragma weak dmx_clip_fwd
#pragma weak dmx_clip_bwd
#pragma weak dmx_declip_project
#pragma weak dmx_hifigan_fwd_dead
#pragma weak dmx_hifigan_dead_plan
#pragma weak dmx_fir_clip_fwd
#pragma weak dmx_fir_clip_bwd
#pragma weak dmx_fir_wgrad
#pragma weak dmx_fir_wgrad_workspace_floats
#pragma weak dmx_ir_update
#pragma weak dmx_stem_mix_fwd
#pragma weak dmx_stem_mix_bwd
#pragma weak dmx_stem_project
#pragma weak dmx_audio_tf_gain
#pragma weak dmx_audio_tf_frames
#pragma weak dmx_audio_tf_curve
#pragma weak dmx_audio_tf_wgrad_segments
#pragma weak dmx_audio_tf_wgrad
#pragma weak dmx_audio_eq_update
#pragma weak dmx_drc_fwd
#pragma weak dmx_drc_bwd

namespace {

#define DMX_DEVICE_OF(t) const c10::hip::HIPGuardMasqueradingAsCUDA dmx_guard_((t).device())
inline void* cur_stream() { return (void*)c10::hip::getCurrentHIPStreamMasqueradingAsCUDA().stream(); }
inline void same_numel(const at::Tensor& a, const at::Tensor& b, const char* what) {
  TORCH_CHECK(a.numel() == b.numel() && a.device() == b.device(), what, ": size / device mismatch");
}

inline void ok(int rc, const char* what) {
  TORCH_CHECK(rc == 0, "diffmusic_hip::", what, " failed with code ", rc, ": ", dmx_last_error());
}
inline void f32_cuda(const at::Tensor& t, const char* name) {
  TORCH_CHECK(t.is_cuda(), name, " must be a GPU tensor (the diffmusic_hip ops have no CPU fallback)");
  TORCH_CHECK(t.scalar_type() == at::kFloat && t.is_contiguous(), name, " must be contiguous fp32");
}
inline void act_cuda(const at::Tensor& t, const char* name) {
// ... 539 lines not shown
  DMX_DEVICE_OF(dmel);
  at::Tensor dz = at::empty({dmel.size(0), latent_channels, dmel.size(1) / scale_factor, dmel.size(2) / scale_factor}, dmel.options().dtype(at::kFloat));
  ok(dmx_vae_decode_bwd(reinterpret_cast<dmx_model*>(model), (const uint16_t*)dmel.data_ptr(), (float)z_scale, dz.data_ptr<float>(), cur_stream()), "vae_dec_bwd");
  return dz;
}
at::Tensor hifigan_fwd(int64_t model, const at::Tensor& mel, at::Tensor ws) {
  act_cuda(mel, "mel");
  DMX_DEVICE_OF(mel);
  dmx_model* m = reinterpret_cast<dmx_model*>(model);
  const int B = (int)mel.size(0), T = (int)mel.size(1);
  at::Tensor wav = at::empty({B, dmx_hifigan_out_len(m, T)}, mel.options().dtype(at::kFloat));
  ok(dmx_hifigan_fwd(m, (const uint16_t*)mel.data_ptr(), wav.data_ptr<float>(), B, T, ws.data_ptr(), ws.nbytes(), cur_stream()), "hifigan_fwd");
  return wav;
}
at::Tensor hifigan_fwd_dead(int64_t model, const at::Tensor& mel, int64_t s0, int64_t s1, at::Tensor ws) {
  act_cuda(mel, "mel");
  DMX_DEVICE_OF(mel);
  dmx_model* m = reinterpret_cast<dmx_model*>(model);
  const int B = (int)mel.size(0), T = (int)mel.size(1);
  at::Tensor wav = at::empty({B, dmx_hifigan_out_len(m, T)}, mel.options().dtype(at::kFloat));
  ok(dmx_hifigan_fwd_dead(m, (const uint16_t*)mel.data_ptr(), wav.data_ptr<float>(), B, T, (int)s0, (int)s1, ws.data_ptr(), ws.nbytes(), cur_stream()),
     "hifigan_fwd_dead");
  return wav;
}
std::vector<int64_t> hifigan_dead_plan(int64_t model, int64_t stages) {
  const int n = (int)stages;
  std::vector<int> a[4];
  for (auto& v : a) v.assign(n > 0 ? n : 1, 0);
  TORCH_CHECK(dmx_hifigan_dead_plan(reinterpret_cast<dmx_model*>(model), a[0].data(), a[1].data(), a[2].data(), a[3].data(), n) >= 0, "hifigan_dead_plan");
  std::vector<int64_t> out;
  for (int s = 0; s < n; ++s) for (auto& v : a) out.push_back(v[s]);
  return out;
}
at::Tensor hifigan_bwd(int64_t model, const at::Tensor& dwav, int64_t frames, int64_t model_in_dim) {
  f32_cuda(dwav, "dwav");
  DMX_DEVICE_OF(dwav);
  at::Tensor dmel = at::empty({dwav.size(0), frames, model_in_dim}, dwav.options().dtype(dmx_act_dtype() == 1 ? at::kHalf : at::kBFloat16));
  ok(dmx_hifigan_bwd(reinterpret_cast<dmx_model*>(model), dwav.data_ptr<float>(), (uint16_t*)dmel.data_ptr(), cur_stream()), "hifigan_bwd");
  return dmel;
}

at::Tensor htsat_fwd(int64_t model, const at::Tensor& mel, bool keep_state, at::Tensor ws) {
  f32_cuda(mel, "mel");
  TORCH_CHECK(mel.dim() == 3, "mel must be (B, frames, mel bins)");
  DMX_DEVICE_OF(mel);
  dmx_model* m = reinterpret_cast<dmx_model*>(model);
  int tokens = 0, channels = 0;
  ok(dmx_htsat_feature_dims(m, &tokens, &channels), "htsat_feature_dims");
  at::Tensor feat = at::empty({mel.size(0), tokens, channels}, mel.options());
  ok(dmx_htsat_fwd(m, mel.data_ptr<float>(), (int)mel.size(0), (int)mel.size(1), feat.data_ptr<float>(), keep_state, ws.data_ptr(), ws.nbytes(),
                   cur_stream()), "htsat_fwd");
  return feat;
}
at::Tensor htsat_bwd(int64_t model, const at::Tensor& dfeat, const std::optional<at::Tensor>& scale, int64_t frames, int64_t bins) {
  f32_cuda(dfeat, "dfeat");
  DMX_DEVICE_OF(dfeat);
  if (scale) { f32_cuda(*scale, "scale"); TORCH_CHECK(scale->numel() == dfeat.size(0) && scale->device() == dfeat.device(), "scale must hold one value per clip"); }
  at::Tensor dmel = at::empty({dfeat.size(0), frames, bins}, dfeat.options());
  ok(dmx_htsat_bwd(reinterpret_cast<dmx_model*>(model), dfeat.data_ptr<float>(), fp(scale), dmel.data_ptr<float>(), cur_stream()), "htsat_bwd");
  return dmel;
}
at::Tensor gram_fwd(const at::Tensor& feat) {
  f32_cuda(feat, "feat");
  TORCH_CHECK(feat.dim() == 3, "feat must be (B, tokens, channels)");
  DMX_DEVICE_OF(feat);
  at::Tensor g = at::empty({feat.size(0), feat.size(2), feat.size(2)}, feat.options());
  ok(dmx_gram_fwd(feat.data_ptr<float>(), g.data_ptr<float>(), (int)feat.size(0), (int)feat.size(1), (int)feat.size(2), cur_stream()), "gram_fwd");
  return g;
}
at::Tensor gram_bwd(const at::Tensor& feat, const at::Tensor& dgram) {
  f32_cuda(feat, "feat"); f32_cuda(dgram, "dgram");
  TORCH_CHECK(feat.dim() == 3 && dgram.numel() == feat.size(0) * feat.size(2) * feat.size(2) && dgram.device() == feat.device(), "dgram must be (B, C, C)");
  DMX_DEVICE_OF(feat);
  at::Tensor d = at::empty_like(feat);
  ok(dmx_gram_bwd(feat.data_ptr<float>(), dgram.data_ptr<float>(), d.data_ptr<float>(), (int)feat.size(0), (int)feat.size(1), (int)feat.size(2), cur_stream()), "gram_bwd");
  return d;
}

}

int64_t abi_version() { return DMX_ABI_VERSION; }

TORCH_LIBRARY(diffmusic_hip, m) {
  TORCH_CHECK(dmx_abi_version() == DMX_ABI_VERSION, "libdiffmusic_torch_ops.so was built against C-ABI version ", DMX_ABI_VERSION,
              " but the loaded libdiffmusic_hip.so reports ", dmx_abi_version(), ": rebuild with `python -m diffmusic_amd.build`");
  {
    const std::pair<const char*, const void*> added[] = {{"dmx_vae_encoder_create", (const void*)&dmx_vae_encoder_create},
                                                         {"dmx_vae_encoder_workspace_bytes", (const void*)&dmx_vae_encoder_workspace_bytes},
                                                         {"dmx_vae_encode_fwd", (const void*)&dmx_vae_encode_fwd},
                                                         {"dmx_latent_init", (const void*)&dmx_latent_init},
                                                         {"dmx_track_stitch_fwd", (const void*)&dmx_track_stitch_fwd},
                                                         {"dmx_track_stitch_bwd", (const void*)&dmx_track_stitch_bwd},
                                                         {"dmx_audio_guidance_fwd_shaped", (const void*)&dmx_audio_guidance_fwd_shaped},
                                                         {"dmx_audio_guidance_bwd_shaped", (const void*)&dmx_audio_guidance_bwd_shaped},
                                                         {"dmx_clip_fwd", (const void*)&dmx_clip_fwd},
                                                         {"dmx_clip_bwd", (const void*)&dmx_clip_bwd},
                                                         {"dmx_declip_project", (const void*)&dmx_declip_project},
                                                         {"dmx_hifigan_fwd_dead", (const void*)&dmx_hifigan_fwd_dead},
                                                         {"dmx_hifigan_dead_plan", (const void*)&dmx_hifigan_dead_plan},
                                                         {"dmx_fir_clip_fwd", (const void*)&dmx_fir_clip_fwd},
                                                         {"dmx_fir_clip_bwd", (const void*)&dmx_fir_clip_bwd},
                                                         {"dmx_fir_wgrad", (const void*)&dmx_fir_wgrad},
                                                         {"dmx_fir_wgrad_workspace_floats", (const void*)&dmx_fir_wgrad_workspace_floats},
                                                         {"dmx_ir_update", (const void*)&dmx_ir_update},
                                                         {"dmx_stem_mix_fwd", (const void*)&dmx_stem_mix_fwd},
                                                         {"dmx_stem_mix_bwd", (const void*)&dmx_stem_mix_bwd},
                                                         {"dmx_stem_project", (const void*)&dmx_stem_project},
                                                         {"dmx_audio_tf_gain", (const void*)&dmx_audio_tf_gain},
                                                         {"dmx_audio_tf_frames", (const void*)&dmx_audio_tf_frames},
                                                         {"dmx_audio_tf_curve", (const void*)&dmx_audio_tf_curve},
                                                         {"dmx_audio_tf_wgrad_segments", (const void*)&dmx_audio_tf_wgrad_segments},
                                                         {"dmx_audio_tf_wgrad", (const void*)&dmx_audio_tf_wgrad},
                                                         {"dmx_audio_eq_update", (const void*)&dmx_audio_eq_update},
                                                         {"dmx_drc_fwd", (const void*)&dmx_drc_fwd},
                                                         {"dmx_drc_bwd", (const void*)&dmx_drc_bwd}};
    for (const auto& s : added)
      TORCH_CHECK(s.second != nullptr, "the loaded libdiffmusic_hip.so reports C-ABI version ", DMX_ABI_VERSION, " but does not export `", s.first,
                  "` (a build from before the VAE encoder / track-mode / declipping / blind-dereverberation / source-separation / time-frequency-masking / blind-equalisation / de-compression entry points): rebuild with `python -m diffmusic_amd.build --force`");
  }
  m.def("abi_version() -> int", &abi_version);
  m.def("sched_pred_x0(Tensor x, Tensor eps, float alpha_t) -> Tensor", &sched_pred_x0);
  m.def("cfg_combine(Tensor eps2, float scale) -> Tensor", &cfg_combine);
  m.def("sched_update(int mode, Tensor x, Tensor eps, Tensor x0, Tensor? g0, Tensor? inv_scale, Tensor? noise, float alpha_t, float alpha_prev, "
        "float sigma, float rate, float eps_small, bool global_norm) -> (Tensor, Tensor?)", &sched_update);
  m.def("randn_philox(int[] shape, int[] seeds, int offset, Device device) -> Tensor", &randn_philox);
  m.def("mask_mul(Tensor x, Tensor? mask, int L, int Ly) -> Tensor", &mask_mul);
  m.def("l2norm(Tensor ref, Tensor pred, float gscale) -> (Tensor, Tensor)", &l2norm);
  m.def("resample_fwd(Tensor x, Tensor h, int Lin, int Lout, int orig, int new_, int off) -> Tensor", &resample_fwd);
  m.def("resample_bwd(Tensor dy, Tensor h, Tensor? h_rev, int Lin, int Lfull, int orig, int new_, int off) -> Tensor", &resample_bwd);
  m.def("fir_clip_fwd(Tensor x, Tensor h, int Lin) -> Tensor", &fir_clip_fwd);
  m.def("fir_clip_bwd(Tensor dy, Tensor h, Tensor h_rev, int Lin, int Lfull) -> Tensor", &fir_clip_bwd);
  m.def("fir_wgrad(Tensor dy, Tensor x, int L, int taps) -> Tensor", &fir_wgrad);
// ... 10 lines not shown
  m.def("clip_fwd(Tensor x, Tensor thr, int L) -> Tensor", &clip_fwd);
  m.def("clip_bwd(Tensor dy, Tensor wav, Tensor thr, int Lfull) -> Tensor", &clip_bwd);
  m.def("declip_project(Tensor wav, Tensor measurement, Tensor thr, int L) -> Tensor", &declip_project);
  m.def("drc_fwd(Tensor x, int L, float threshold_db, float slope, float knee_db, float a_att, float a_rel, float makeup_db) -> (Tensor, Tensor, Tensor)",
        &drc_fwd);
  m.def("drc_bwd(Tensor dy, Tensor x, Tensor state, Tensor tape, int Lfull, float threshold_db, float slope, float knee_db, float a_att, float a_rel, "
        "float makeup_db) -> Tensor", &drc_bwd);
  m.def("noise_add(Tensor y, Tensor noise, float sigma) -> Tensor", &noise_add);
  m.def("tf_gain(int audio, Tensor x, Tensor gain_t, int L, int Lfull) -> Tensor", &tf_gain);
  m.def("tf_curve(int audio, Tensor x, Tensor curve, int L, int Lfull) -> Tensor", &tf_curve);
  m.def("tf_wgrad(int audio, Tensor dy, Tensor x, int L) -> Tensor", &tf_wgrad);
  m.def("eq_update(Tensor partials, Tensor(a!) g, Tensor(b!) m, Tensor(c!) v, int k, float lr, float beta1, float beta2, float eps, bool peak) "
        "-> ()", &eq_update);
  m.def("track_stitch_fwd(Tensor wav, int[] starts, int L, int R, int T) -> Tensor", &track_stitch_fwd);
  m.def("track_stitch_bwd(Tensor dtrack, int[] starts, int L, int R, int Lfull) -> Tensor", &track_stitch_bwd);
  m.def("stem_mix_fwd(Tensor wav, float[]? gains, int K, int G, int L) -> Tensor", &stem_mix_fwd);
  m.def("stem_mix_bwd(Tensor dmix, float[]? gains, int K, int Lfull) -> Tensor", &stem_mix_bwd);
  m.def("stem_project(Tensor x, Tensor y, float[]? gains, int L) -> Tensor", &stem_project);
  m.def("stft_mag_fwd(int audio, Tensor wav, Tensor(a!) state, int L) -> Tensor", &stft_mag_fwd);
  m.def("stft_mag_bwd(int audio, Tensor dmag, Tensor state, int L, int Lfull) -> Tensor", &stft_mag_bwd);
  m.def("melscale_fwd(int audio, Tensor mag, float lo, float hi) -> Tensor", &melscale_fwd);
  m.def("unet_fwd(int model, Tensor x, Tensor t, Tensor? class_labels, Tensor(a!) ws) -> Tensor", &unet_fwd);
  m.def("unet_fwd_ctx(int model, Tensor x, Tensor t, Tensor? class_labels, Tensor c0, Tensor c1, Tensor bias1, Tensor(a!) ws) -> Tensor", &unet_fwd_ctx);
  m.def("vae_dec_fwd(int model, Tensor z, float z_scale, bool keep_state, bool want_f32, int scale_factor, Tensor(a!) ws) -> (Tensor, Tensor?)", &vae_dec_fwd);
  m.def("vae_dec_bwd(int model, Tensor dmel, float z_scale, int latent_channels, int scale_factor) -> Tensor", &vae_dec_bwd);
  m.def("vae_enc_fwd(int model, Tensor mel, float log_floor, int latent_channels, int scale_factor, Tensor(a!) ws) -> Tensor", &vae_enc_fwd);
  m.def("latent_init(Tensor moments, int h, int w, Tensor? eps, Tensor? noise, float sqrt_abar, float scaling_factor, float sqrt_1m_abar, "
        "bool want_x) -> (Tensor, Tensor, Tensor?)", &latent_init);
  m.def("grad_normalize_(Tensor(a!) dwav, float target) -> Tensor", &grad_normalize_);
  m.def("hifigan_fwd(int model, Tensor mel, Tensor(a!) ws) -> Tensor", &hifigan_fwd);
  m.def("hifigan_bwd(int model, Tensor dwav, int frames, int model_in_dim) -> Tensor", &hifigan_bwd);
  m.def("hifigan_fwd_dead(int model, Tensor mel, int s0, int s1, Tensor(a!) ws) -> Tensor", &hifigan_fwd_dead);
  m.def("hifigan_dead_plan(int model, int stages) -> int[]", &hifigan_dead_plan);
  m.def("htsat_fwd(int model, Tensor mel, bool keep_state, Tensor(a!) ws) -> Tensor", &htsat_fwd);
  m.def("htsat_bwd(int model, Tensor dfeat, Tensor? scale, int frames, int bins) -> Tensor", &htsat_bwd);
  m.def("gram_fwd(Tensor feat) -> Tensor", &gram_fwd);
  m.def("gram_bwd(Tensor feat, Tensor dgram) -> Tensor", &gram_bwd);
}
```

diffmusic_amd/engine.py:

```python
import ctypes as C
import os
import torch
from . import _lib as L
from . import ops
from ._ctypes_ops import _stream
from .weights import synth_state_dict

HIFIGAN_DEFAULT = dict(model_in_dim=64, upsample_initial_channel=1024, upsample_rates=[5, 4, 2, 2, 2],
                       upsample_kernel_sizes=[16, 16, 8, 4, 4], resblock_kernel_sizes=[3, 7, 11],
                       resblock_dilation_sizes=[[1, 3, 5]] * 3, leaky_relu_slope=0.1, sampling_rate=16000)
VAE_DEFAULT = dict(latent_channels=8, out_channels=1, block_out_channels=[128, 256, 512], layers_per_block=2,
                   norm_num_groups=32, scaling_factor=0.9227914214134216, eps=1e-6)
UNET_MUSICLDM_DEFAULT = dict(in_channels=8, out_channels=8, block_out_channels=[128, 256, 384, 640],
                             layers_per_block=2, attention_heads=8, norm_num_groups=32,
                             down_attn=[0, 1, 1, 1], up_attn=[1, 1, 1, 0], class_embed_dim=512, attn_cross_dims=[0])
UNET_AUDIOLDM2_DEFAULT = dict(UNET_MUSICLDM_DEFAULT, class_embed_dim=0, attn_cross_dims=[0, 768, 1024])


def _fill(arr, vals):
    for i, v in enumerate(vals):
        arr[i] = int(v)


class _Engine:
# ... 46 lines not shown
            L.check(lib.dmx_model_finalize(self._h, _stream()), "finalize")
            torch.cuda.synchronize()
        self._finalized = True
        return self

    def _workspace(self, key, nbytes):
        ws = self._ws.get("buf")
        if ws is None or ws.numel() < nbytes:
            self._ws.clear()
            ws = torch.empty(int(nbytes), dtype=torch.uint8, device=self.device)
            self._ws["buf"] = ws
        return ws


class HifiGanEngine(_Engine):
    kind = "hifigan"
    allow_unexpected = ("mean", "scale")

    def __init__(self, config=None, device="cuda"):
        cfg = dict(HIFIGAN_DEFAULT)
        cfg.update(config or {})
        c = L.HifiGanConfig()
        c.model_in_dim, c.upsample_initial_channel = cfg["model_in_dim"], cfg["upsample_initial_channel"]
        c.num_upsamples = len(cfg["upsample_rates"])
        _fill(c.upsample_rates, cfg["upsample_rates"])
        _fill(c.upsample_kernel_sizes, cfg["upsample_kernel_sizes"])
        c.num_kernels = len(cfg["resblock_kernel_sizes"])
        _fill(c.resblock_kernel_sizes, cfg["resblock_kernel_sizes"])
        c.num_dilations = len(cfg["resblock_dilation_sizes"][0])
        _fill(c.resblock_dilation_sizes, [d for row in cfg["resblock_dilation_sizes"] for d in row])
        c.leaky_relu_slope = cfg["leaky_relu_slope"]
        super().__init__(L.lib().dmx_hifigan_create(C.byref(c)), cfg, device)
        self.dead_span_enabled = os.environ.get("DMX_NO_DEAD_SPAN", "0") in ("", "0")

    def _stride_of(self, name):
        return self.cfg["upsample_rates"][int(name.split(".")[1])]

    @property
    def config(self):
        from types import SimpleNamespace
        return SimpleNamespace(**self.cfg)

    def out_len(self, frames):
        return L.lib().dmx_hifigan_out_len(self._h, frames)

    def __call__(self, mel):
        return self.forward(mel.to(device=self.device, dtype=L.act_dtype()).contiguous())

    def forward(self, mel, dead=None):
        assert mel.dtype == L.act_dtype() and mel.is_cuda and mel.is_contiguous()
        B, T, _ = mel.shape
        lib = L.lib()
        ws = self._workspace(("h", B, T), lib.dmx_hifigan_workspace_bytes(self._h, B, T))
        self._shape = (B, T)
        if dead is not None and self.dead_span_enabled and int(dead[1]) > int(dead[0]):
            return ops.hip.hifigan_fwd_dead(self._h.value, mel, int(dead[0]), int(dead[1]), ws)
        return ops.hip.hifigan_fwd(self._h.value, mel, ws)

    def dead_plan(self):
        n = len(self.cfg["upsample_rates"])
        flat = list(ops.hip.hifigan_dead_plan(self._h.value, n))
        return [dict(skipped=flat[4 * s], total=flat[4 * s + 1], span=(flat[4 * s + 2], flat[4 * s + 3])) for s in range(n)]

    def backward(self, dwav):
        _, T = self._shape
        assert dwav.dtype == torch.float32 and dwav.is_contiguous()
        return ops.hip.hifigan_bwd(self._h.value, dwav, T, self.cfg["model_in_dim"])


class VaeDecoderEngine(_Engine):
    kind = "vae"
    allow_unexpected = ("encoder.", "quant_conv.")

    def __init__(self, config=None, device="cuda"):
        cfg = dict(VAE_DEFAULT)
        cfg.update(config or {})
        c = L.VaeConfig()
        c.latent_channels, c.out_channels = cfg["latent_channels"], cfg["out_channels"]
        c.num_blocks = len(cfg["block_out_channels"])
        _fill(c.block_out_channels, cfg["block_out_channels"])
        c.layers_per_block, c.norm_num_groups, c.eps = cfg["layers_per_block"], cfg["norm_num_groups"], cfg["eps"]
        super().__init__(L.lib().dmx_vae_decoder_create(C.byref(c)), cfg, device)
        self.scale_factor = 2 ** (c.num_blocks - 1)
        self.scaling_factor = cfg["scaling_factor"]

    @property
    def config(self):
        from types import SimpleNamespace
        return SimpleNamespace(**self.cfg)

    def decode(self, z):
        from types import SimpleNamespace
        _, m32 = self.decode_hip(z.to(device=self.device, dtype=torch.float32).contiguous(), 1.0, keep_state=False, want_f32=True)
        return SimpleNamespace(sample=m32.unsqueeze(1))

# ... 186 lines not shown
```

include/diffmusic_hip.h:

```cpp
#ifndef DIFFMUSIC_HIP_H
#define DIFFMUSIC_HIP_H
#include <stddef.h>
#include <stdint.h>

#ifdef __cplusplus
extern "C" {
#endif

#define DMX_ABI_VERSION 4
#define DMX_MAX_STAGES 8

typedef struct dmx_model dmx_model;

typedef struct dmx_hifigan_config {
  int model_in_dim;
  int upsample_initial_channel;
  int num_upsamples;
  int upsample_rates[DMX_MAX_STAGES];
  int upsample_kernel_sizes[DMX_MAX_STAGES];
  int num_kernels;
  int resblock_kernel_sizes[DMX_MAX_STAGES];
  int num_dilations;
  int resblock_dilation_sizes[DMX_MAX_STAGES * DMX_MAX_STAGES];
  float leaky_relu_slope;
// ... 17 lines not shown
  int attention_heads;
  int norm_num_groups;
  int down_attn[DMX_MAX_STAGES];
  int up_attn[DMX_MAX_STAGES];
  int class_embed_dim;
  int num_attn_per_layer;
  int attn_cross_dims[4];
} dmx_unet_config;

int dmx_abi_version(void);
int dmx_act_dtype(void);
const char* dmx_last_error(void);

dmx_model* dmx_hifigan_create(const dmx_hifigan_config* cfg);
dmx_model* dmx_vae_decoder_create(const dmx_vae_config* cfg);
dmx_model* dmx_unet_create(const dmx_unet_config* cfg);
void dmx_model_destroy(dmx_model* m);
int dmx_model_num_params(const dmx_model* m);
const char* dmx_model_param_name(const dmx_model* m, int i);
size_t dmx_model_param_numel(const dmx_model* m, int i);
int dmx_model_param_ndim(const dmx_model* m, int i);
int dmx_model_param_dim(const dmx_model* m, int i, int d);
int dmx_model_load_param(dmx_model* m, const char* name, const float* data_host, size_t numel);
int dmx_model_finalize(dmx_model* m, void* stream);

int dmx_hifigan_out_len(const dmx_model* m, int frames);
size_t dmx_hifigan_workspace_bytes(dmx_model* m, int batch, int frames);
int dmx_hifigan_fwd(dmx_model* m, const uint16_t* mel, float* wav, int batch, int frames, void* ws, size_t ws_bytes,
                    void* stream);
int dmx_hifigan_bwd(dmx_model* m, const float* dwav, uint16_t* dmel, void* stream);
int dmx_hifigan_fwd_dead(dmx_model* m, const uint16_t* mel, float* wav, int batch, int frames, int s0, int s1, void* ws,
                         size_t ws_bytes, void* stream);
int dmx_hifigan_dead_plan(dmx_model* m, int* skipped, int* total, int* lo, int* hi, int n);
int dmx_conv_dead_rows(int k, int dil, int pad, int stride, int transposed, int t_in, int t_out, int a, int b, int* lo, int* hi);

size_t dmx_vae_workspace_bytes(dmx_model* m, int batch, int h, int w);
int dmx_vae_decode_fwd(dmx_model* m, const float* z, float z_scale, uint16_t* mel, float* mel_f32, int batch, int h, int w,
                       int keep_state, void* ws, size_t ws_bytes, void* stream);
int dmx_vae_decode_bwd(dmx_model* m, const uint16_t* dmel, float z_scale, float* dz, void* stream);

dmx_model* dmx_vae_encoder_create(const dmx_vae_config* cfg);
size_t dmx_vae_encoder_workspace_bytes(dmx_model* m, int batch, int frames, int bins);
int dmx_vae_encode_fwd(dmx_model* m, const float* mel, float log_floor, float* moments, int batch, int frames, int bins, void* ws,
                       size_t ws_bytes, void* stream);
int dmx_latent_init(const float* moments, float* mean, float* logvar, float* x, const float* eps, const float* noise, int batch,
                    int latent_channels, int hw, float sqrt_abar, float scaling_factor, float sqrt_1m_abar, void* stream);

size_t dmx_unet_workspace_bytes(dmx_model* m, int batch, int h, int w);
int dmx_unet_fwd(dmx_model* m, const float* x, const float* t, const float* class_labels, float* eps, int batch, int h,
                 int w, void* ws, size_t ws_bytes, void* stream);
int dmx_unet_fwd_ctx(dmx_model* m, const float* x, const float* t, const float* class_labels, const float* ctx0, int n0,
                     const float* ctx1, int n1, const float* bias1, float* eps, int batch, int h, int w, void* ws,
                     size_t ws_bytes, void* stream);
size_t dmx_unet_workspace_bytes_ctx(dmx_model* m, int batch, int h, int w, int n0, int n1);

typedef struct dmx_htsat_config {
  int spec_size;
  int num_mel_bins;
  int patch_size;
  int embed_dim;
  int window_size;
  int num_stages;
  int depths[4];
  int num_heads[4];
  float ln_eps;
  float bn_eps;
// ... 83 lines not shown
int dmx_fir_clip_fwd(const float* in, long long in_stride, const float* h, float* out, long long out_stride, int batch, int Lin, int Lout,
                     int taps, void* stream);
int dmx_fir_clip_bwd(const float* dout, long long dout_stride, const float* h, const float* h_rev, float* din, long long din_stride, int batch,
                     int Lin, int Lout, int taps, void* stream);
size_t dmx_fir_wgrad_workspace_floats(int batch, int Lout, int taps);
int dmx_fir_wgrad(const float* dy, long long dy_stride, const float* x, long long x_stride, float* partials, size_t partial_floats, int batch,
                  int L, int Lout, int taps, void* stream);
int dmx_ir_update(const float* partials, int segments, float* h, float* h_rev, float* m, float* v, int batch, int taps, double lr, double beta1,
                  double beta2, double eps, int k, void* stream);

#define DMX_SCHED_DDIM 0
#define DMX_SCHED_DPS 1
#define DMX_SCHED_MPGD 2
#define DMX_SCHED_DSG 3
#define DMX_SCHED_DIFFMUSIC 4
int dmx_sched_pred_x0(const float* x, const float* eps, float* x0, long long n, float alpha_t, void* stream);
int dmx_sched_pred_x0_ex(const float* x, const float* model_output, float* x0, long long n, float alpha_t, int prediction_type, float clip_range,
                         void* stream);
int dmx_sched_cfg_combine(const float* eps2, float* out, long long n, float scale, void* stream);
int dmx_sched_step(int mode, const float* x, const float* eps, const float* x0, const float* g0, const float* inv_scale,
                   const float* noise, float* prev, float* x0_out, float* grad_out, int batch, int n, float alpha_t, float alpha_prev,
                   float sigma, float rate, float eps_small, int global_norm, void* stream);
int dmx_sched_step_ex(int mode, const float* x, const float* eps, const float* x0, const float* g0, const float* inv_scale,
                      const float* noise, float* prev, float* x0_out, float* grad_out, int batch, int n, float alpha_t, float alpha_prev,
                      float sigma, float rate, float eps_small, int global_norm, int prediction_type, float clip_range, void* stream);

int dmx_randn_philox(float* out, int batch, long long n, const unsigned long long* seeds_host, unsigned long long offset, void* stream);

void dmx_prof_begin(void);
int dmx_prof_end(double* total_ms, double* total_flops);
int dmx_prof_dominant(double* ms, double* flops, double* bytes);

int dmx_gemm_raw(const void* desc, size_t desc_bytes, void* stream);
int dmx_flash_attn_raw(const void* q, const void* k, const void* v, void* o, const float* colbias, int B, int Nq, int Nk, int ldv,
                       int C, int heads, float scale, void* stream);
int dmx_flash_attn_ld_raw(const void* q, const void* k, const void* v, void* o, const float* colbias, int B, int Nq, int Nk, int ldq,
                          int ldk, int ldv, int C, int heads, float scale, int* qt_out, void* stream);
int dmx_softmax_raw(const float* S, void* P, const float* colbias, long long rows, int N, long long lds, long long ldp, int rows_per_bias,
                    void* stream);
int dmx_softmax_act_raw(const void* S, void* P, const float* colbias, long long rows, int N, long long ldp, int rows_per_bias, void* stream);
int dmx_transpose_raw(const void* in, void* out, int R, int C, long long ldi, long long ldo, int Z, int Zi, long long sIo, long long sIi,
                      long long sOo, long long sOi, void* stream);
int dmx_rowdot_raw(const void* a, const void* b, float* out, long long rows, int C, long long lda, long long ldb, void* stream);
int dmx_layernorm_raw(const void* x, void* y, const float* gamma, const float* beta, int rows, int C, float eps, void* stream);
int dmx_geglu_raw(const void* x, void* y, long long rows, int I, void* stream);
int dmx_gemm_splitk_workspace(void* ws, size_t bytes);
int dmx_conv_pair_raw(const void* desc_a, const void* desc_b, size_t desc_bytes, void* stream);
int dmx_conv_pair_dead_raw(const void* desc_a, const void* desc_b, size_t desc_bytes, const int* dead, int* skipped, int* total, void* stream);
int dmx_conv_pair_group_raw(int n, const void* descs_a, const void* descs_b, size_t desc_bytes, void* stream);
int dmx_conv_pair_group_dead_raw(int n, const void* descs_a, const void* descs_b, size_t desc_bytes, const int* dead, void* stream);
size_t dmx_groupnorm_scratch_floats(int B, int C, int G);
int dmx_groupnorm_raw(const void* x, void* y, const float* gamma, const float* beta, float* stats, float* scale, float* shift,
                      float* partial, int B, int P, int C, int G, float eps, int silu, void* stream);
size_t dmx_groupnorm_part_floats(int B, int P, int N);
int dmx_groupnorm_parts_raw(const void* x, void* y, const float* gamma, const float* beta, float* stats, float* scale, float* shift,
                            int B, int P, int C, int G, float eps, int silu, int nreg, float* const* part, const int* geom, void* stream);
int dmx_gemm_last_tile_rows_raw(void);
int dmx_conv2d_raw(const float* w_host, const float* b_host, const void* x, void* y, int B, int Hi, int Wi, int Ci, int Co, int k, int stride,
                   int pad_lo, int pad_hi, void* stream);
int dmx_groupnorm_bwd_raw(const void* x, const void* dy, const void* add, void* dx, const float* stats, const float* scale, const float* shift,
                          float* k0, float* k1, float* partial, int B, int P, int C, int G, int silu, int nreg, float* const* part,
                          const int* geom, void* stream);

#ifdef __cplusplus
}
#endif
// ... 2 lines not shown
```

Baseline: 26.79 steps/s (weak scaling: one step advances a batch of 8 clips on one GPU; value = K / wall x 1 GPU(s)).

## Compact dead rows in HiFi-GAN 1-D conv GEMMs via row-gap mapping

Adds a row-compacted GEMM path for whole-clip stride-1 1-D convolutions in HiFi-GAN. It drops the contiguous time span whose output is known dead (the inpainting gap) from the M dimension and remaps rows in the epilogue, zero-filling the rows that must be cleared. A cost model decides per launch whether the compacted tile config beats the plain one, with an auto mode on by default. The aim is to avoid computing conv rows that are discarded anyway. In exchange it adds epilogue index math, a new tile config (288-row), and dirty-row clearing that could be wrong at the gap boundaries.

```diff
diff --git a/diffmusic_amd/_ctypes_ops.py b/diffmusic_amd/_ctypes_ops.py
--- a/diffmusic_amd/_ctypes_ops.py
+++ b/diffmusic_amd/_ctypes_ops.py
@@ -517,6 +517,21 @@
     return [int(a[s]) for s in range(n) for a in arr]
 
 
+def hifigan_dead_rows(model, stages):
+    n = int(stages)
+    arr = [(C.c_int * n)() for _ in range(2)]
+    if _lib.lib().dmx_hifigan_dead_rows(model, *arr, n) < 0:
+        _lib.check(-1, "hifigan_dead_rows")
+    return [int(a[s]) for s in range(n) for a in arr]
+
+
+def hifigan_set_dead_rows(model, mode):
+    prev = _lib.lib().dmx_hifigan_set_dead_rows(model, int(mode))
+    if prev < 0:
+        _lib.check(-1, "hifigan_set_dead_rows")
+    return int(prev)
+
+
 def hifigan_bwd(model, dwav, frames, model_in_dim):
     dmel = torch.empty(dwav.shape[0], frames, model_in_dim, dtype=_lib.act_dtype(), device=dwav.device)
     _lib.check(_lib.lib().dmx_hifigan_bwd(model, _p(dwav), _p(dmel), _stream()), "hifigan_bwd")
diff --git a/diffmusic_amd/_lib.py b/diffmusic_amd/_lib.py
--- a/diffmusic_amd/_lib.py
+++ b/diffmusic_amd/_lib.py
@@ -82,6 +82,10 @@
                                        C.c_void_p]),
     "dmx_hifigan_dead_plan": (C.c_int, [C.c_void_p, C.POINTER(C.c_int), C.POINTER(C.c_int), C.POINTER(C.c_int), C.POINTER(C.c_int), C.c_int]),
     "dmx_conv_dead_rows": (C.c_int, [C.c_int] * 9 + [C.POINTER(C.c_int), C.POINTER(C.c_int)]),
+    "dmx_hifigan_set_dead_rows": (C.c_int, [C.c_void_p, C.c_int]),
+    "dmx_hifigan_dead_rows": (C.c_int, [C.c_void_p, C.POINTER(C.c_int), C.POINTER(C.c_int), C.c_int]),
+    "dmx_gemm_rows_plan": (C.c_int, [C.c_int] * 5 + [C.POINTER(C.c_int), C.POINTER(C.c_int)]),
+    "dmx_gemm_rows_raw": (C.c_int, [C.c_void_p, C.c_size_t, C.POINTER(C.c_int), C.c_int, C.c_void_p]),
     "dmx_vae_workspace_bytes": (C.c_size_t, [C.c_void_p, C.c_int, C.c_int, C.c_int]),
     "dmx_vae_decode_fwd": (C.c_int, [C.c_void_p, C.c_void_p, C.c_float, C.c_void_p, C.c_void_p, C.c_int, C.c_int, C.c_int,
                                      C.c_int, C.c_void_p, C.c_size_t, C.c_void_p]),
@@ -206,7 +210,8 @@
                "dmx_clip_fwd", "dmx_clip_bwd", "dmx_declip_project", "dmx_hifigan_fwd_dead", "dmx_hifigan_dead_plan", "dmx_conv_dead_rows",
                "dmx_fir_clip_fwd", "dmx_fir_clip_bwd", "dmx_fir_wgrad", "dmx_fir_wgrad_workspace_floats", "dmx_ir_update",
                "dmx_stem_mix_fwd", "dmx_stem_mix_bwd", "dmx_stem_project", "dmx_audio_tf_gain", "dmx_audio_tf_frames",
-               "dmx_audio_tf_curve", "dmx_audio_tf_wgrad_segments", "dmx_audio_tf_wgrad", "dmx_audio_eq_update", "dmx_drc_fwd", "dmx_drc_bwd")
+               "dmx_audio_tf_curve", "dmx_audio_tf_wgrad_segments", "dmx_audio_tf_wgrad", "dmx_audio_eq_update", "dmx_drc_fwd", "dmx_drc_bwd",
+               "dmx_hifigan_set_dead_rows", "dmx_hifigan_dead_rows", "dmx_gemm_rows_plan", "dmx_gemm_rows_raw")
 
 _lib = None
 
@@ -215,7 +220,7 @@
     for name in ADDED_IN_V4:
         if not hasattr(h, name):
             raise RuntimeError(f"{path} reports ABI version {ABI_VERSION} but does not export `{name}` (a build from before the VAE "
-                               "encoder / track-mode / declipping / blind-dereverberation / source-separation / time-frequency-masking / blind-equalisation / de-compression entry points): rebuild it (python -m diffmusic_amd.build --force)")
+                               "encoder / track-mode / declipping / blind-dereverberation / source-separation / time-frequency-masking / blind-equalisation / de-compression / dead-row compaction entry points): rebuild it (python -m diffmusic_amd.build --force)")
 
 
 def lib():
diff --git a/diffmusic_amd/csrc/capi.hip b/diffmusic_amd/csrc/capi.hip
--- a/diffmusic_amd/csrc/capi.hip
+++ b/diffmusic_amd/csrc/capi.hip
@@ -72,6 +72,27 @@
 int dmx_hifigan_dead_plan(dmx_model* m, int* skipped, int* total, int* lo, int* hi, int n) {
   if (!m || !m->impl || m->impl->kind != DMX_MODEL_HIFIGAN) { dmx_set_error("wrong model handle"); return -1; }
   return dmx_hifigan_dead_plan_impl(m->impl, skipped, total, lo, hi, n);
+}
+int dmx_hifigan_dead_rows(dmx_model* m, int* rows, int* launches, int n) {
+  if (!m || !m->impl || m->impl->kind != DMX_MODEL_HIFIGAN) { dmx_set_error("wrong model handle"); return -1; }
+  return dmx_hifigan_dead_rows_impl(m->impl, rows, launches, n);
+}
+int dmx_hifigan_set_dead_rows(dmx_model* m, int mode) {
+  if (!m || !m->impl || m->impl->kind != DMX_MODEL_HIFIGAN) { dmx_set_error("wrong model handle"); return -1; }
+  if (mode < 0 || mode > 2) { dmx_set_error("hifigan_set_dead_rows: mode 0 (off), 1 (auto) or 2 (force)"); return -1; }
+  return dmx_hifigan_set_dead_rows_impl(m->impl, mode);
+}
+int dmx_gemm_rows_plan(int M, int live_M, int N, int K, int mode, int* cfg, int* tiles) {
+  return dmx_gemm_rows_plan_impl(M, live_M, N, K, mode, cfg, tiles);
+}
+int dmx_gemm_rows_raw(const void* desc, size_t desc_bytes, const int* gap, int cfg, void* stream) {
+  if (desc_bytes != sizeof(GemmDesc)) { dmx_set_error("GemmDesc size mismatch: %zu vs %zu", desc_bytes, sizeof(GemmDesc)); return DMX_ERR_SHAPE; }
+  if (!gap) return DMX_ERR_STATE;
+  RowGap rg;
+  rg.g0 = gap[1]; rg.gn = gap[2]; rg.z0 = gap[3]; rg.z1 = gap[4]; rg.rz0 = gap[5]; rg.rz1 = gap[6];
+  const int rc = dmx_gemm_launch_rows(*reinterpret_cast<const GemmDesc*>(desc), rg, cfg, ST(stream));
+  if (rc == DMX_ERR_SHAPE) dmx_set_error("gemm_rows: not a whole-clip stride-1 1-D convolution with the 16-bit epilogue, a gap outside the clip, or a tile without row map");
+  return rc;
 }
 int dmx_conv_dead_rows(int k, int dil, int pad, int stride, int transposed, int t_in, int t_out, int a, int b, int* lo, int* hi) {
   if (!lo || !hi) return DMX_ERR_STATE;
diff --git a/diffmusic_amd/csrc/dmx_common.h b/diffmusic_amd/csrc/dmx_common.h
--- a/diffmusic_amd/csrc/dmx_common.h
+++ b/diffmusic_amd/csrc/dmx_common.h
@@ -139,6 +139,12 @@
   int gnb_cpg;
 };
 
+struct RowGap { int Wl = 0, g0 = 0, gn = 0, z0 = 0, z1 = 0, rz0 = 0, rz1 = 0; };
+int dmx_gemm_launch_rows_cfg(int cfg, const GemmDesc& d, const RowGap& rg, hipStream_t stream);
+int dmx_gemm_launch_rows(const GemmDesc& d, const RowGap& rg, int cfg, hipStream_t stream);
+bool dmx_gemm_rows_eligible(const GemmDesc& d);
+int dmx_gemm_rows_plan_impl(int M, int live_M, int N, int K, int mode, int* cfg, int* tiles);
+
 int dmx_gemm_launch(const GemmDesc& d, hipStream_t stream, int* gn_rows = nullptr);
 void dmx_gemm_set_splitk_workspace(float* ws, size_t bytes);
 void dmx_gemm_release_splitk_workspace(const float* ws);
diff --git a/diffmusic_amd/csrc/gemm_conv.hip b/diffmusic_amd/csrc/gemm_conv.hip
--- a/diffmusic_amd/csrc/gemm_conv.hip
+++ b/diffmusic_amd/csrc/gemm_conv.hip
@@ -37,6 +37,42 @@
 static const TileEntry g_tile_table[] = {
 #include "tile_table.inc"
     {0, 0, 0, 0, 0}};
+
+struct Cand { int cfg, bm, bn, slots; double eff; bool rows; };
+const Cand g_cands[] = {{1, 256, 256, 256, 0.95, true}, {7, 320, 256, 256, 0.93, true}, {8, 192, 256, 256, 0.88, false},
+                        {2, 256, 128, 256, 0.70, false}, {9, 320, 128, 256, 0.70, false}, {10, 192, 128, 256, 0.66, false},
+                        {19, 512, 128, 256, 0.75, false},
+                        {3, 128, 128, 512, 0.66, false}};
+const Cand g_cand288 = {20, 288, 256, 256, 0.93, true};
+double tile_cost(const Cand& c, int M, int N, int Z) {
+  const double blocks = (double)cdiv(M, c.bm) * cdiv(N, c.bn) * Z;
+  const double rounds = ceil(blocks / c.slots);
+  return rounds * (c.bm / 128.0) * (c.bn / 128.0) * (c.slots / 256.0) / c.eff;
+}
+int model_pick(int M, int N, int Z, double* cost_out) {
+  int best = 0;
+  double bc = 1e30;
+  for (const Cand& c : g_cands) {
+    if (c.bn == 256 && N % 256) continue;
+    const double v = tile_cost(c, M, N, Z);
+    if (v < bc) { bc = v; best = c.cfg; }
+  }
+  if (cost_out) *cost_out = bc;
+  return best;
+}
+int rows_pick(int M, int N, double* cost_out, int* tiles) {
+  int best = 0;
+  double bc = 1e30;
+  auto take = [&](const Cand& c) {
+    if (!c.rows) return;
+    const double v = tile_cost(c, M, N, 1);
+    if (v < bc) { bc = v; best = c.cfg; if (tiles) *tiles = cdiv(M, c.bm) * cdiv(N, c.bn); }
+  };
+  for (const Cand& c : g_cands) take(c);
+  take(g_cand288);
+  if (cost_out) *cost_out = bc;
+  return best;
+}
 
 bool glds_ok(const GemmDesc& d) {
   const long long imgs = d.Hq * d.Wq > 0 ? (d.M + (long long)d.Hq * d.Wq - 1) / ((long long)d.Hq * d.Wq) : 1;
@@ -98,23 +134,7 @@
       if ((c > 2 && c < 7) || gl) return launch_by_cfg(c, d, stream, gn_rows);
     }
   if (gl && d.M >= 2048 && d.N % 128 == 0) {
-    auto cost = [&](int bm, int bn, int slots, double eff) {
-      const double blocks = (double)cdiv(d.M, bm) * cdiv(d.N, bn) * d.Z;
-      const double rounds = ceil(blocks / slots);
-      return rounds * (bm / 128.0) * (bn / 128.0) * (slots / 256.0) / eff;
-    };
-    struct Cand { int cfg, bm, bn, slots; double eff; };
-    static const Cand cands[] = {{1, 256, 256, 256, 0.95}, {7, 320, 256, 256, 0.93}, {8, 192, 256, 256, 0.88},
-                                 {2, 256, 128, 256, 0.70}, {9, 320, 128, 256, 0.70}, {10, 192, 128, 256, 0.66},
-                                 {19, 512, 128, 256, 0.75},
-                                 {3, 128, 128, 512, 0.66}};
-    int best = 0;
-    double bc = 1e30;
-    for (const Cand& c : cands) {
-      if (c.bn == 256 && d.N % 256) continue;
-      const double v = cost(c.bm, c.bn, c.slots, c.eff);
-      if (v < bc) { bc = v; best = c.cfg; }
-    }
+    const int best = model_pick(d.M, d.N, d.Z, nullptr);
     if (best && best != 3) return launch_by_cfg(best, d, stream, gn_rows);
   }
   if (d.N > 32 && (long long)cdiv(d.M, 128) * cdiv(d.N, 128) * d.Z < 200) {
@@ -159,7 +179,7 @@
     float t = 0.f;
     if (hipEventElapsedTime(&t, r.a, r.b) == hipSuccess) ms += t;
     if (csv) fprintf(csv, "%d,%d,%d,%d,%d,%d,%d,%.4f,%.1f\n", r.M, r.N, r.K, r.Z, r.taps, r.flags, r.cfg, t, t > 0 ? r.flops / t / 1e9 : 0.0);
-    const bool dma = r.cfg == 1 || r.cfg == 2 || (r.cfg >= 7 && r.cfg <= 10) || r.cfg == 19;
+    const bool dma = r.cfg == 1 || r.cfg == 2 || (r.cfg >= 7 && r.cfg <= 10) || r.cfg == 19 || r.cfg == 20;
     if (dma) { g_dma_ms += t; g_dma_fl += r.flops; g_dma_by += r.bytes; ++g_dma_n; }
     fl += r.flops;
     (void)hipEventDestroy(r.a); (void)hipEventDestroy(r.b);
@@ -286,6 +306,79 @@
   r.flops = flops; r.bytes = bytes; r.M = M; r.N = N; r.K = K; r.Z = 1; r.taps = taps; r.flags = flags; r.cfg = cfg;
 }
 
+int dmx_gemm_rows_plan_impl(int M, int live_M, int N, int K, int mode, int* cfg, int* tiles) {
+  int plain = 0;
+  double plain_cost = 0.0;
+  for (const TileEntry* e = g_tile_table; e->cfg; ++e)
+    if (e->M == M && e->N == N && e->K == K && e->Z == 1 && !plain) plain = e->cfg % 100;
+  const bool modelled = !plain && M >= 2048 && N > 0 && N % 128 == 0;
+  if (modelled) plain = model_pick(M, N, 1, &plain_cost);
+  else if (plain)
+    for (const Cand& c : g_cands) if (c.cfg == plain) plain_cost = tile_cost(c, M, N, 1);
+  if (cfg) *cfg = plain;
+  if (tiles) *tiles = 0;
+  if (mode <= 0 || live_M <= 0 || live_M >= M || N <= 0 || (N & 7)) return 0;
+  double c = 0.0;
+  int t = 0;
+  const int best = rows_pick(live_M, N, &c, &t);
+  if (!best) return 0;
+  if (mode == 1 && !(plain_cost > 0.0 && N % 256 == 0 && c < plain_cost)) return 0;
+  if (cfg) *cfg = best;
+  if (tiles) *tiles = t;
+  return 1;
+}
+
+bool dmx_gemm_rows_eligible(const GemmDesc& d) {
+  if (d.M <= 0 || d.N <= 0 || d.K <= 0 || (d.Ci & 7) || (d.K & 7) || (d.lda & 7) || (d.ldw & 7)) return false;
+  if (d.ntaps < 1 || d.ntaps > DMX_MAX_TAPS || d.K != d.ntaps * d.Ci) return false;
+  if (d.Z != 1 || d.Zi != 1 || d.Hq != 1 || d.Hi != 1 || d.Ho != 1 || d.sx != 1 || d.sy != 1 || d.osx != 1 || d.osy != 1 || d.oox || d.ooy) return false;
+  if (d.Wq < 1 || d.Wo != d.Wq || d.M % d.Wq) return false;
+  for (int t = 0; t < d.ntaps; ++t) if (d.tdy[t]) return false;
+  if (d.flags & ~(EPI_BIAS | EPI_RESID | EPI_RESID_INV | EPI_ACCUM | EPI_MASK | EPI_LRELU2 | EPI_NO_C)) return false;
+  if ((d.N | d.ldc | d.ldr | d.ldx | d.ldc2) & 7) return false;
+  if ((d.flags & EPI_LRELU2) && !(d.act_slope >= 0.f && d.act_slope <= 1.f)) return false;
+  if ((d.flags & EPI_RESID_INV) && !(d.resid_inv_slope >= 1.f)) return false;
+  if (d.tile_cfg >= 100 || !glds_ok(d)) return false;
+  int kt = 12;
+  return splitk_plan(d, &kt) <= 1;
+}
+
+int dmx_gemm_launch_rows(const GemmDesc& d, const RowGap& rg, int cfg, hipStream_t stream) {
+  if (!dmx_gemm_rows_eligible(d)) return DMX_ERR_SHAPE;
+  if (rg.g0 < 0 || rg.gn < 0 || rg.gn >= d.Wq || rg.g0 + rg.gn > d.Wq) return DMX_ERR_SHAPE;
+  RowGap r = rg;
+  r.Wl = d.Wq - rg.gn;
+  if (r.z1 <= r.z0) r.z0 = r.z1 = 0;
+  if (r.rz1 <= r.rz0) r.rz0 = r.rz1 = 0;
+  GemmDesc q = d;
+  q.M = d.M / d.Wq * r.Wl;
+  q.tile_cfg = 0;
+  if (!cfg) cfg = rows_pick(q.M, q.N, nullptr, nullptr);
+  if (cfg != 1 && cfg != 7 && cfg != 20) return DMX_ERR_SHAPE;
+  g_last_cfg = cfg;
+  if (!g_prof) return dmx_gemm_launch_rows_cfg(cfg, q, r, stream);
+  ProfRec pr;
+  memset(&pr, 0, sizeof(pr));
+  (void)hipEventCreate(&pr.a); (void)hipEventCreate(&pr.b);
+  pr.flops = 2.0 * q.M * (double)q.N * q.K;
+  {
+    const double mn = (double)q.M * q.N;
+    double by = 2.0 * q.M * (double)q.Ci + 2.0 * q.N * (double)q.K;
+    if (!(q.flags & EPI_NO_C)) by += mn * 2.0;
+    if (q.flags & EPI_ACCUM) by += mn * 2.0;
+    if (q.flags & (EPI_RESID | EPI_RESID_INV)) by += mn * 2.0;
+    if (q.flags & EPI_MASK) by += mn * 2.0;
+    if (q.C2 && (q.flags & EPI_LRELU2)) by += mn * 2.0;
+    pr.bytes = by;
+  }
+  pr.M = q.M; pr.N = q.N; pr.K = q.K; pr.Z = 1; pr.taps = q.ntaps; pr.flags = q.flags; pr.cfg = cfg;
+  (void)hipEventRecord(pr.a, stream);
+  const int rc = dmx_gemm_launch_rows_cfg(cfg, q, r, stream);
+  (void)hipEventRecord(pr.b, stream);
+  g_prof_recs.push_back(pr);
+  return rc;
+}
+
 int dmx_gemm_launch(const GemmDesc& d, hipStream_t stream, int* gn_rows) {
   if (gn_rows) *gn_rows = 0;
   if (d.M <= 0 || d.N <= 0 || d.K <= 0) return DMX_ERR_SHAPE;
diff --git a/diffmusic_amd/csrc/gemm_epilogue.h b/diffmusic_amd/csrc/gemm_epilogue.h
--- a/diffmusic_amd/csrc/gemm_epilogue.h
+++ b/diffmusic_amd/csrc/gemm_epilogue.h
@@ -98,10 +98,10 @@
 template <int FM>
 struct EpiChunk { static constexpr int IB = (FM % DMX_EPI_IB == 0) ? DMX_EPI_IB : (FM % 4 == 0) ? 4 : (FM % 3 == 0) ? 3 : (FM % 2 == 0) ? 2 : 1; static constexpr int CH = IB * 16; };
 
-template <int FM, int FN, int EM>
+template <int FM, int FN, int EM, bool RC = false>
 __device__ __forceinline__ void gemm_epilogue_lds_impl(const GemmDesc& p, f32x4 (&acc)[FM][FN], int m0, int n0, int lane,
                                                        long long coff, int HqWq, char* wl, int mlimit,
-                                                       const uint2 (&rpre)[FM * FN], const bool use_rpre) {
+                                                       const uint2 (&rpre)[FM * FN], const bool use_rpre, const RowGap rg = RowGap{}) {
   constexpr bool BITS = EM == 1;
   constexpr bool SOFT = EM == 2;
   constexpr bool GEGLU = EM == 3;
@@ -109,6 +109,8 @@
   static_assert(!ROWS || FN == 2 || FN == 4, "row statistics come in slots of 32 columns");
   constexpr bool GNS = EM == 5;
   constexpr bool GNB = EM == 6;
+  static_assert(!RC || EM == 0, "row compaction: the plain 16-bit epilogue only");
+  constexpr int RZ_FLAG = 1 << 30;
   static_assert(!GEGLU || FN % 2 == 0, "GEGLU pairs accumulator fragments");
   constexpr int CH = EpiChunk<FM>::CH;
   constexpr int IB = EpiChunk<FM>::IB;
@@ -125,7 +127,7 @@
   const int ncol = n0 + cch * 8;
   const bool col_ok = ncol < p.N;
   const int mend = p.M < mlimit ? p.M : mlimit;
-  const bool ident = p.osy == 1 && p.osx == 1 && p.ooy == 0 && p.oox == 0 && p.Ho == p.Hq && p.Wo == p.Wq;
+  const bool ident = !RC && p.osy == 1 && p.osx == 1 && p.ooy == 0 && p.oox == 0 && p.Ho == p.Hq && p.Wo == p.Wq;
 #define DMX_LDS_SYNC() asm volatile("s_waitcnt lgkmcnt(0)" ::: "memory")
   float4 bcol[FN];
 #pragma unroll
@@ -140,6 +142,7 @@
   static_for<0, FM / IB>([&](auto H) {
     constexpr int h = decltype(H)::value;
     int orows[NIT];
+    bool rzero[RC ? NIT : 1];
     if (ident) {
 #pragma unroll
       for (int it = 0; it < NIT; ++it) {
@@ -150,6 +153,14 @@
       if (lane < CH) {
         const int m = m0 + h * CH + lane;
         int orow = -1;
+        if constexpr (RC) {
+          if (m < mend) {
+            const int b = m / rg.Wl;
+            int t = m - b * rg.Wl;
+            if (t >= rg.g0) t += rg.gn;
+            orow = (b * p.Wo + t) | ((t >= rg.rz0 && t < rg.rz1) ? RZ_FLAG : 0);
+          }
+        } else
         if (m < mend) {
           const int b = m / HqWq, rem = m - b * HqWq;
           const int qy = rem / p.Wq, qx = rem - qy * p.Wq;
@@ -160,14 +171,22 @@
       DMX_LDS_SYNC();
 #pragma unroll
       for (int it = 0; it < NIT; ++it) orows[it] = tab[it * RPI + rr];
-      DMX_LDS_SYNC();
-    }
-    auto stage_in = [&](const act_t* G, int ld, auto&& f) {
+      if constexpr (RC) {
+#pragma unroll
+        for (int it = 0; it < NIT; ++it) {
+          rzero[it] = orows[it] >= 0 && (orows[it] & RZ_FLAG) != 0;
+          if (orows[it] >= 0) orows[it] &= ~RZ_FLAG;
+        }
+      }
+      DMX_LDS_SYNC();
+    }
+    auto stage_in = [&](const act_t* G, int ld, auto&& f, const bool resid = false) {
       {
         uint4 v[NIT];
 #pragma unroll
         for (int it = 0; it < NIT; ++it) {
-          const bool ok = orows[it] >= 0 && col_ok;
+          bool ok = orows[it] >= 0 && col_ok;
+          if constexpr (RC) ok = ok && !(resid && rzero[it]);
           const long long off = ok ? (long long)orows[it] * ld + ncol : 0ll;
           v[it] = *reinterpret_cast<const uint4*>(G + coff + off);
           if (!ok) v[it] = make_uint4(0, 0, 0, 0);
@@ -409,7 +428,7 @@
       const float is = (flags & EPI_RESID_INV) ? p.resid_inv_slope : 1.f;
       stage_in(p.R, p.ldr, [&](f32x4& a, float x0, float x1, float x2, float x3) {
         a[0] += fminf(x0, x0 * is); a[1] += fminf(x1, x1 * is); a[2] += fminf(x2, x2 * is); a[3] += fminf(x3, x3 * is);
-      });
+      }, true);
     }
     if (p.alpha != 1.f) {
       const float al = p.alpha;
@@ -488,11 +507,11 @@
 #undef DMX_LDS_SYNC
 }
 
-template <int FM, int FN, int EM>
+template <int FM, int FN, int EM, bool RC = false>
 __device__ __forceinline__ void gemm_epilogue_lds(const GemmDesc& p, f32x4 (&acc)[FM][FN], int m0, int n0, int lane,
-                                                  long long coff, int HqWq, char* wl, int mlimit = 0x7fffffff) {
+                                                  long long coff, int HqWq, char* wl, int mlimit = 0x7fffffff, const RowGap rg = RowGap{}) {
   const uint2 none[FM * FN] = {};
-  gemm_epilogue_lds_impl<FM, FN, EM>(p, acc, m0, n0, lane, coff, HqWq, wl, mlimit, none, false);
+  gemm_epilogue_lds_impl<FM, FN, EM, RC>(p, acc, m0, n0, lane, coff, HqWq, wl, mlimit, none, false, rg);
 }
 
 }
diff --git a/diffmusic_amd/csrc/gemm_rows.hip b/diffmusic_amd/csrc/gemm_rows.hip
--- /dev/null
+++ b/diffmusic_amd/csrc/gemm_rows.hip
@@ -0,0 +1,42 @@
+#include "gemm_tile.h"
+
+namespace {
+
+template <int BM, int BN, int WM, int WN, int NSTAGE, int BMF>
+__global__ __launch_bounds__(WM* WN * 64) void gemm_glds_rows_kernel(const GemmDesc p, const RowGap rg) {
+  extern __shared__ __attribute__((aligned(16))) char smem[];
+  const int tiles_n = (p.N + BN - 1) / BN;
+  const int bid = xcd_remap(blockIdx.x);
+  glds_tile<BM, BN, WM, WN, NSTAGE, 0, false, BMF, true>(p, smem, (bid / tiles_n) * BM, bid % tiles_n, p.M, rg);
+}
+
+template <int BM, int BN, int WM, int WN, int NSTAGE, int BMF>
+int launch_rows_t(const GemmDesc& d, const RowGap& rg, hipStream_t stream) {
+  constexpr int NT = WM * WN * 64;
+  constexpr int SMEM = NSTAGE * (BMF + BN) * 128;
+  static_assert(SMEM <= 160 * 1024, "tile ring exceeds the 160 KiB of LDS");
+  static bool attr_set = false;
+  if (!attr_set) {
+    hipFuncSetAttribute(reinterpret_cast<const void*>(&gemm_glds_rows_kernel<BM, BN, WM, WN, NSTAGE, BMF>),
+                        hipFuncAttributeMaxDynamicSharedMemorySize, SMEM);
+    attr_set = true;
+  }
+  const long long tiles = (long long)cdiv(d.M, BM) * cdiv(d.N, BN);
+  GemmDesc q = d;
+  static const bool bias_init = getenv("DMX_NO_BIAS_INIT") == nullptr;
+  if (bias_init && (d.flags & EPI_BIAS) && d.bias && !(d.flags & (EPI_MASK | EPI_MASKBITS | EPI_SOFTBWD | EPI_LNFOLD)))
+    q.flags = (q.flags & ~EPI_BIAS) | EPI_BIASINIT;
+  hipLaunchKernelGGL((gemm_glds_rows_kernel<BM, BN, WM, WN, NSTAGE, BMF>), dim3((unsigned)tiles, 1, 1), dim3(NT), SMEM, stream, q, rg);
+  return hipGetLastError() == hipSuccess ? DMX_OK : DMX_ERR_LAUNCH;
+}
+
+}
+
+int dmx_gemm_launch_rows_cfg(int cfg, const GemmDesc& d, const RowGap& rg, hipStream_t stream) {
+  switch (cfg) {
+    case 1: return launch_rows_t<256, 256, 2, 4, 2, 256>(d, rg, stream);
+    case 7: return launch_rows_t<320, 256, 2, 4, 2, 320>(d, rg, stream);
+    case 20: return launch_rows_t<288, 256, 2, 4, 2, 320>(d, rg, stream);
+    default: return DMX_ERR_SHAPE;
+  }
+}
diff --git a/diffmusic_amd/csrc/gemm_tile.h b/diffmusic_amd/csrc/gemm_tile.h
--- a/diffmusic_amd/csrc/gemm_tile.h
+++ b/diffmusic_amd/csrc/gemm_tile.h
@@ -232,14 +232,16 @@
 #define DMX_GSTAMP(i) do { } while (0)
 #endif
 
-template <int BM, int BN, int WM, int WN, int NSTAGE, int EM, bool LNF = false>
-__device__ __forceinline__ void glds_tile(const GemmDesc& p, char* smem, const int m0, const int tn, const int mlim) {
+template <int BM, int BN, int WM, int WN, int NSTAGE, int EM, bool LNF = false, int BMF = BM, bool RC = false>
+__device__ __forceinline__ void glds_tile(const GemmDesc& p, char* smem, const int m0, const int tn, const int mlim, const RowGap rg = RowGap{}) {
   constexpr int NW = WM * WN;
   constexpr int TM = BM / WM, TN = BN / WN;
   constexpr int FM = TM / 16, FN = TN / 16;
-  constexpr int A_ISS = BM / 8 / NW, B_ISS = BN / 8 / NW;
-  constexpr int A_BYTES = BM * 128, B_BYTES = BN * 128, STAGE = A_BYTES + B_BYTES;
+  constexpr int A_ISS = BMF / 8 / NW, B_ISS = BN / 8 / NW;
+  constexpr int A_BYTES = BMF * 128, B_BYTES = BN * 128, STAGE = A_BYTES + B_BYTES;
   static_assert(A_ISS >= 1 && B_ISS >= 1, "tile too small");
+  static_assert(BMF >= BM && BMF % (8 * NW) == 0 && TM % 16 == 0, "the A stage holds whole rounds of LDS-DMA instructions");
+  static_assert(!RC || (EM == 0 && !LNF), "row compaction: the plain 16-bit epilogue only");
 
   constexpr int PER = A_ISS + B_ISS;
   constexpr int KEEP = (NSTAGE - 2) * PER;
@@ -277,8 +279,12 @@
       const int m = m0 + (i * NW + wave) * 8 + lrow;
       r_mask[i] = 0u; a_lin[i] = 0u;
       r_iy[i] = -(1 << 20); r_ix[i] = 0;
-      if (m < mlim) {
+      if (m < mlim && (BMF == BM || m < m0 + BM)) {
         int b = 0, qy = 0, qx = m;
+        if constexpr (RC) {
+          b = m / rg.Wl; qx = m - b * rg.Wl;
+          if (qx >= rg.g0) qx += rg.gn;
+        } else
         if (!(p.Hq == 1 && p.Wq >= p.M)) {
           b = m / HqWq; const int rem = m - b * HqWq;
           qy = rem / p.Wq; qx = rem - qy * p.Wq;
@@ -292,7 +298,9 @@
       const int dy = (int)(signed char)(tv & 0xff), dx = (int)(signed char)((tv >> 8) & 0xff);
 #pragma unroll
       for (int i = 0; i < A_ISS; ++i)
-        if ((unsigned)(r_iy[i] + dy) < (unsigned)p.Hi && (unsigned)(r_ix[i] + dx) < (unsigned)p.Wi) r_mask[i] |= 1u << t;
+        if ((unsigned)(r_iy[i] + dy) < (unsigned)p.Hi && (unsigned)(r_ix[i] + dx) < (unsigned)p.Wi &&
+            !(RC && r_ix[i] + dx >= rg.z0 && r_ix[i] + dx < rg.z1))
+          r_mask[i] |= 1u << t;
     }
 #pragma unroll
     for (int i = 0; i < (A_ISS + 1) / 2; ++i) a_mask2[i] = 0u;
@@ -497,6 +505,12 @@
   __builtin_amdgcn_s_barrier();
   DMX_GSTAMP(2);
   if constexpr (LNF) ln_apply<FM, FN, BN>(acc, s_ln, s_cs, wm * TM, wn * TN, lr, lq);
+  if constexpr (RC) {
+    constexpr int EPI_CH = EpiChunk<FM>::CH;
+    constexpr int EPI_WAVE_BYTES = EPI_CH * (FN * 32 + 16) + EPI_CH * 12;
+    static_assert(EPI_WAVE_BYTES * WM * WN <= 2 * (BM + BN) * 128, "epilogue staging does not fit the stage buffers");
+    gemm_epilogue_lds<FM, FN, EM, true>(p, acc, m0 + wm * TM, tn * BN + wn * TN, lane, coff, HqWq, smem + wave * EPI_WAVE_BYTES, mlim, rg);
+  } else
   if ((p.flags & EPI_F32OUT) || ((p.N | p.ldc | p.ldr | p.ldx | p.ldc2) & 7)) {
     gemm_epilogue<FM, FN>(p, acc, m0 + wm * TM, tn * BN + wn * TN, lr, lq, coff, HqWq);
   } else {
diff --git a/diffmusic_amd/csrc/hifigan.hip b/diffmusic_amd/csrc/hifigan.hip
--- a/diffmusic_amd/csrc/hifigan.hip
+++ b/diffmusic_amd/csrc/hifigan.hip
@@ -1,6 +1,7 @@
 #include "models.h"
 #include "conv_pair.h"
 #include <cstdlib>
+#include <cstring>
 
 struct SplitKScope {
   explicit SplitKScope(float* ws, size_t bytes, bool on) : on_(on && ws) { if (on_) dmx_gemm_set_splitk_workspace(ws, bytes); }
@@ -48,12 +49,23 @@
   std::vector<Span> out, xs;
   std::vector<Span> xo, h, x;
   std::vector<int> skipped, total;
+  int rows_mode = 0;
+  bool rows_on = false;
 };
 
 struct HifiGan : Model {
   dmx_hifigan_config cfg;
   DeadPlan plan;
   bool use_dead = false;
+  int rows_mode = 1;
+  std::vector<int> rows_cnt[2], rows_launches[2];
+  struct DirtyRows { const void* p; Span s; };
+  std::vector<DirtyRows> dirty;
+  Span dirty_of(const void* p) const { for (const DirtyRows& d : dirty) if (d.p == p) return d.s; return Span{}; }
+  void set_dirty(const void* p, Span sp) {
+    for (size_t i = 0; i < dirty.size(); ++i) if (dirty[i].p == p) { dirty.erase(dirty.begin() + i); break; }
+    if (p && !sp.empty()) dirty.push_back(DirtyRows{p, sp});
+  }
   static constexpr size_t kSplitKBytes = 32u << 20;
   float* splitk_ws = nullptr;
   ConvLayer conv_pre, conv_post;
@@ -108,6 +120,7 @@
     events.resize(256);
     for (auto& e : events) (void)hipEventCreateWithFlags(&e, hipEventDisableTiming);
     splitk_ws = (float*)ps.dalloc(kSplitKBytes);
+    if (const char* e = getenv("DMX_DEAD_ROWS")) rows_mode = (!strcmp(e, "off") || !strcmp(e, "0")) ? 0 : (!strcmp(e, "force") ? 2 : 1);
   }
   ~HifiGan() override {
     dmx_gemm_release_splitk_workspace(splitk_ws);
@@ -169,9 +182,9 @@
   }
 
   void make_plan(int T_, int s0, int s1) {
-    if (plan.B == B && plan.T == T_ && plan.s0 == s0 && plan.s1 == s1 && (int)plan.out.size() == ns) return;
+    if (plan.B == B && plan.T == T_ && plan.s0 == s0 && plan.s1 == s1 && plan.rows_mode == rows_mode && (int)plan.out.size() == ns) return;
     plan = DeadPlan();
-    plan.B = B; plan.T = T_; plan.s0 = s0; plan.s1 = s1;
+    plan.B = B; plan.T = T_; plan.s0 = s0; plan.s1 = s1; plan.rows_mode = rows_mode;
     plan.out.assign(ns, Span{}); plan.xs.assign(ns, Span{});
     plan.xo.assign(ns * nk * nd, Span{}); plan.h.assign(ns * nk * nd, Span{}); plan.x.assign(ns * nk * nd, Span{});
     plan.skipped.assign(ns, 0); plan.total.assign(ns, 0);
@@ -203,7 +216,19 @@
     if (multi_wanted()) return;
     int any = 0;
     for (int s = 0; s < ns; ++s) {
-      if (!stage_all_fused(s, len[s])) continue;
+      if (!stage_all_fused(s, len[s])) {
+        bool none = true;
+        for (int k = 0; k < nk; ++k) for (int d = 0; d < nd; ++d) none = none && !step_is_fused(idx(s, k, d), len[s]);
+        if (!none || rows_mode <= 0) continue;
+        for (int k = 0; k < nk; ++k)
+          for (int d = 0; d < nd; ++d) {
+            const int id = idx(s, k, d), C = ups[s].Cop, K = c1[id].kw * C;
+            const Span w[3] = {plan.h[id], plan.xo[id], d == 0 ? plan.xs[s] : plan.x[id]};
+            for (const Span& sp : w)
+              if (!sp.empty() && dmx_gemm_rows_plan_impl(B * len[s], B * (len[s] - (sp.b - sp.a)), C, K, rows_mode, nullptr, nullptr)) plan.rows_on = true;
+          }
+        continue;
+      }
       for (int k = 0; k < nk; ++k)
         for (int d = 0; d < nd; ++d) {
           const int id = idx(s, k, d);
@@ -219,6 +244,54 @@
     if (!plan.on) plan.skipped.assign(ns, 0);
   }
 
+  int clear_dirty(const void* t, int rows, int ld, hipStream_t st) {
+    const Span sp = dirty_of(t);
+    if (sp.empty()) return DMX_OK;
+    if (hipMemset2DAsync((act_t*)const_cast<void*>(t) + (size_t)sp.a * ld, (size_t)rows * ld * sizeof(act_t), 0, (size_t)(sp.b - sp.a) * ld * sizeof(act_t),
+                         (size_t)B, st) != hipSuccess) {
+      dmx_set_error("hifigan: clearing the dead rows of a gradient failed");
+      return DMX_ERR_LAUNCH;
+    }
+    set_dirty(t, Span{});
+    return DMX_OK;
+  }
+  int run_rows(const GemmDesc& d, Span skip, bool bwd, int s, hipStream_t st) {
+    const Span zA = bwd ? dirty_of(d.A) : Span{};
+    const Span zR = bwd && (d.flags & EPI_RESID) ? dirty_of(d.R) : Span{};
+    const bool elig = dmx_gemm_rows_eligible(d);
+    int cfg = 0;
+    bool compact = false;
+    if (elig && !skip.empty()) {
+      const int clips = d.M / d.Wq;
+      compact = dmx_gemm_rows_plan_impl(d.M, d.M - clips * (skip.b - skip.a), d.N, d.K, rows_mode, &cfg, nullptr) == 1;
+    }
+    void* c_out = (d.flags & EPI_NO_C) ? nullptr : d.C;
+    void* c2_out = (d.flags & EPI_LRELU2) ? (void*)d.C2 : nullptr;
+    const Span c_prev = (d.flags & EPI_ACCUM) ? dirty_of(d.C) : Span{};
+    RowGap rg;
+    rg.z0 = zA.a; rg.z1 = zA.b; rg.rz0 = zR.a; rg.rz1 = zR.b;
+    if (compact) {
+      rg.g0 = skip.a; rg.gn = skip.b - skip.a;
+      RUN(dmx_gemm_launch_rows(d, rg, cfg, st));
+      rows_cnt[bwd][s] += rg.gn; rows_launches[bwd][s] += 1;
+      if (bwd) { set_dirty(c_out, skip); set_dirty(c2_out, skip); }
+      return DMX_OK;
+    }
+    if (!zA.empty() || !zR.empty()) {
+      if (elig) {
+        RUN(dmx_gemm_launch_rows(d, rg, 0, st));
+      } else {
+        RUN(clear_dirty(d.A, d.Wi, d.lda, st));
+        if (d.flags & EPI_RESID) RUN(clear_dirty(d.R, d.Wo, d.ldr, st));
+        RUN(dmx_gemm_launch(d, st));
+      }
+    } else {
+      RUN(dmx_gemm_launch(d, st));
+    }
+    if (bwd) { set_dirty(c_out, c_prev); set_dirty(c2_out, Span{}); }
+    return DMX_OK;
+  }
+
   int out_len(int T_) const {
     int t = T_;
     for (int i = 0; i < ns; ++i) t = conv_out_len(ups[i], t);
@@ -231,7 +304,9 @@
     B = B_;
     if (!dry) {
       use_dead = false;
-      if (s1 > s0) { make_plan(T_, s0, s1); use_dead = plan.on; }
+      if (s1 > s0) { make_plan(T_, s0, s1); use_dead = plan.on || plan.rows_on; }
+      for (auto& v : rows_cnt) v.assign(ns, 0);
+      for (auto& v : rows_launches) v.assign(ns, 0);
     }
     const bool dead = use_dead && !dry;
     SplitKScope sk_scope(splitk_ws, kSplitKBytes, !dry && !multi_wanted());
@@ -329,6 +404,8 @@
         (void)hipEventRecord(e0, st);
         for (int k = 1; k < nk; ++k) (void)hipStreamWaitEvent(bstream[k], e0, 0);
       }
+      bool none_fused = true;
+      for (int k = 0; k < nk; ++k) for (int d = 0; d < nd; ++d) none_fused = none_fused && fused[idx(s, k, d)] == 0;
       for (int k = 0; k < nk; ++k) {
         hipStream_t sk = (mt && k > 0) ? bstream[k] : st;
         for (int d = 0; d < nd; ++d) {
@@ -358,6 +435,10 @@
             return DMX_ERR_STATE;
           }
           if (d == nd - 1 && mt && fin_prev) (void)hipStreamWaitEvent(sk, fin_prev, 0);
+          if (dead && !mt && none_fused && rows_mode > 0) {
+            RUN(run_rows(da, plan.h[id], false, s, sk));
+            RUN(run_rows(db, plan.xo[id], false, s, sk));
+          } else
           RUN(conv_pair_run(da, db, sk));
           if (d == nd - 1 && mt) { fin_prev = next_event(); (void)hipEventRecord(fin_prev, sk); }
         }
@@ -391,6 +472,8 @@
     act_t* g = arena.bf((size_t)B * Tout * Clast);
     CHECK_WS("hifigan");
     const bool dead = use_dead && !dry;
+    dirty.clear();
+    if (!dry) { rows_cnt[1].assign(ns, 0); rows_launches[1].assign(ns, 0); }
     if (dead) RUN(dmx_tanh_bwd_pad8_dead(dwav, wav8, gz, (long long)B * Tout, Tout, plan.wav.a, plan.wav.b, st));
     else RUN(dmx_tanh_bwd_pad8(dwav, wav8, gz, (long long)B * Tout, st));
     {
@@ -450,6 +533,8 @@
         (void)hipEventRecord(e0, st);
         for (int k = 1; k < nk; ++k) (void)hipStreamWaitEvent(bstream[k], e0, 0);
       }
+      bool none_fused = true;
+      for (int k = 0; k < nk; ++k) for (int d = 0; d < nd; ++d) none_fused = none_fused && fused[idx(s, k, d)] == 0;
       for (int k = 0; k < nk; ++k) {
         hipStream_t sk = (mt && k > 0) ? bstream[k] : st;
         const act_t* gc = g;
@@ -472,6 +557,10 @@
             dst = (gc == gAB[k][0]) ? gAB[k][1] : gAB[k][0];
           }
           RUN(conv_bwd_1d_desc(c1[id], ghk[k], dst, B, To, e, db));
+          if (dead && !mt && none_fused && rows_mode > 0) {
+            RUN(run_rows(da, plan.h[id], true, s, sk));
+            RUN(run_rows(db, d == 0 ? plan.xs[s] : plan.x[id], true, s, sk));
+          } else
           RUN(conv_pair_run(da, db, sk));
           if (d == 0 && mt) { fin_prev = next_event(); (void)hipEventRecord(fin_prev, sk); }
           gc = dst;
@@ -479,6 +568,7 @@
       }
       }
       if (mt && fin_prev) (void)hipStreamWaitEvent(st, fin_prev, 0);
+      if (!dry) RUN(clear_dirty(gxs, To, C, st));
       {
         Epi e; e.flags = EPI_MASK; e.mask_slope = slope;
         if (s > 0) { e.X = act_out[s - 1]; e.alpha = 1.f / nk; } else { e.X = act_pre; }
@@ -514,6 +604,23 @@
   }
   return h->ns;
 }
+int dmx_hifigan_dead_rows_impl(Model* m, int* rows, int* launches, int n) {
+  HifiGan* h = static_cast<HifiGan*>(m);
+  for (int s = 0; s < n && s < h->ns; ++s) {
+    int r = 0, l = 0;
+    for (int dir = 0; dir < 2; ++dir)
+      if (h->use_dead && s < (int)h->rows_cnt[dir].size()) { r += h->rows_cnt[dir][s]; l += h->rows_launches[dir][s]; }
+    if (rows) rows[s] = r;
+    if (launches) launches[s] = l;
+  }
+  return h->ns;
+}
+int dmx_hifigan_set_dead_rows_impl(Model* m, int mode) {
+  HifiGan* h = static_cast<HifiGan*>(m);
+  const int prev = h->rows_mode;
+  if (mode >= 0 && mode <= 2) h->rows_mode = mode;
+  return prev;
+}
 int dmx_hifigan_bwd_impl(Model* m, const float* dwav, act_t* dmel, hipStream_t st) {
   return static_cast<HifiGan*>(m)->backward(dwav, dmel, st);
 }
diff --git a/diffmusic_amd/csrc/models.h b/diffmusic_amd/csrc/models.h
--- a/diffmusic_amd/csrc/models.h
+++ b/diffmusic_amd/csrc/models.h
@@ -24,6 +24,8 @@
 int dmx_hifigan_bwd_impl(Model* m, const float* dwav, act_t* dmel, hipStream_t st);
 int dmx_hifigan_fwd_dead_impl(Model* m, const act_t* mel, float* wav, int B, int T, int s0, int s1, void* ws, size_t wsb, hipStream_t st);
 int dmx_hifigan_dead_plan_impl(Model* m, int* skipped, int* total, int* lo, int* hi, int n);
+int dmx_hifigan_dead_rows_impl(Model* m, int* rows, int* launches, int n);
+int dmx_hifigan_set_dead_rows_impl(Model* m, int mode);
 int dmx_conv_dead_rows_impl(int k, int dil, int pad, int stride, int transposed, int t_in, int t_out, int a, int b, int* lo, int* hi);
 size_t dmx_hifigan_ws_impl(Model* m, int B, int T);
 
diff --git a/diffmusic_amd/csrc_torch/torch_ops.cpp b/diffmusic_amd/csrc_torch/torch_ops.cpp
--- a/diffmusic_amd/csrc_torch/torch_ops.cpp
+++ b/diffmusic_amd/csrc_torch/torch_ops.cpp
@@ -19,6 +19,8 @@
 #pragma weak dmx_declip_project
 #pragma weak dmx_hifigan_fwd_dead
 #pragma weak dmx_hifigan_dead_plan
+#pragma weak dmx_hifigan_dead_rows
+#pragma weak dmx_hifigan_set_dead_rows
 #pragma weak dmx_fir_clip_fwd
 #pragma weak dmx_fir_clip_bwd
 #pragma weak dmx_fir_wgrad
@@ -624,6 +626,20 @@
   for (int s = 0; s < n; ++s) for (auto& v : a) out.push_back(v[s]);
   return out;
 }
+std::vector<int64_t> hifigan_dead_rows(int64_t model, int64_t stages) {
+  const int n = (int)stages;
+  std::vector<int> a[2];
+  for (auto& v : a) v.assign(n > 0 ? n : 1, 0);
+  TORCH_CHECK(dmx_hifigan_dead_rows(reinterpret_cast<dmx_model*>(model), a[0].data(), a[1].data(), n) >= 0, "hifigan_dead_rows");
+  std::vector<int64_t> out;
+  for (int s = 0; s < n; ++s) for (auto& v : a) out.push_back(v[s]);
+  return out;
+}
+int64_t hifigan_set_dead_rows(int64_t model, int64_t mode) {
+  const int prev = dmx_hifigan_set_dead_rows(reinterpret_cast<dmx_model*>(model), (int)mode);
+  TORCH_CHECK(prev >= 0, "hifigan_set_dead_rows: ", dmx_last_error());
+  return prev;
+}
 at::Tensor hifigan_bwd(int64_t model, const at::Tensor& dwav, int64_t frames, int64_t model_in_dim) {
   f32_cuda(dwav, "dwav");
   DMX_DEVICE_OF(dwav);
@@ -690,6 +706,8 @@
                                                          {"dmx_declip_project", (const void*)&dmx_declip_project},
                                                          {"dmx_hifigan_fwd_dead", (const void*)&dmx_hifigan_fwd_dead},
                                                          {"dmx_hifigan_dead_plan", (const void*)&dmx_hifigan_dead_plan},
+                                                         {"dmx_hifigan_dead_rows", (const void*)&dmx_hifigan_dead_rows},
+                                                         {"dmx_hifigan_set_dead_rows", (const void*)&dmx_hifigan_set_dead_rows},
                                                          {"dmx_fir_clip_fwd", (const void*)&dmx_fir_clip_fwd},
                                                          {"dmx_fir_clip_bwd", (const void*)&dmx_fir_clip_bwd},
                                                          {"dmx_fir_wgrad", (const void*)&dmx_fir_wgrad},
@@ -766,6 +784,8 @@
   m.def("hifigan_bwd(int model, Tensor dwav, int frames, int model_in_dim) -> Tensor", &hifigan_bwd);
   m.def("hifigan_fwd_dead(int model, Tensor mel, int s0, int s1, Tensor(a!) ws) -> Tensor", &hifigan_fwd_dead);
   m.def("hifigan_dead_plan(int model, int stages) -> int[]", &hifigan_dead_plan);
+  m.def("hifigan_dead_rows(int model, int stages) -> int[]", &hifigan_dead_rows);
+  m.def("hifigan_set_dead_rows(int model, int mode) -> int", &hifigan_set_dead_rows);
   m.def("htsat_fwd(int model, Tensor mel, bool keep_state, Tensor(a!) ws) -> Tensor", &htsat_fwd);
   m.def("htsat_bwd(int model, Tensor dfeat, Tensor? scale, int frames, int bins) -> Tensor", &htsat_bwd);
   m.def("gram_fwd(Tensor feat) -> Tensor", &gram_fwd);
diff --git a/diffmusic_amd/engine.py b/diffmusic_amd/engine.py
--- a/diffmusic_amd/engine.py
+++ b/diffmusic_amd/engine.py
@@ -102,6 +102,7 @@
         c.leaky_relu_slope = cfg["leaky_relu_slope"]
         super().__init__(L.lib().dmx_hifigan_create(C.byref(c)), cfg, device)
         self.dead_span_enabled = os.environ.get("DMX_NO_DEAD_SPAN", "0") in ("", "0")
+        self.dead_rows = os.environ.get("DMX_DEAD_ROWS", "") or "auto"
 
     def _stride_of(self, name):
         return self.cfg["upsample_rates"][int(name.split(".")[1])]
@@ -131,6 +132,25 @@
         n = len(self.cfg["upsample_rates"])
         flat = list(ops.hip.hifigan_dead_plan(self._h.value, n))
         return [dict(skipped=flat[4 * s], total=flat[4 * s + 1], span=(flat[4 * s + 2], flat[4 * s + 3])) for s in range(n)]
+
+    DEAD_ROWS_MODES = ("off", "auto", "force")
+
+    @property
+    def dead_rows(self):
+        return self._dead_rows
+
+    @dead_rows.setter
+    def dead_rows(self, mode):
+        mode = {"0": "off"}.get(mode, mode)
+        if mode not in self.DEAD_ROWS_MODES:
+            raise ValueError(f"dead_rows must be one of {self.DEAD_ROWS_MODES}, not {mode!r}")
+        ops.hip.hifigan_set_dead_rows(self._h.value, self.DEAD_ROWS_MODES.index(mode))
+        self._dead_rows = mode
+
+    def dead_rows_report(self):
+        n = len(self.cfg["upsample_rates"])
+        flat = list(ops.hip.hifigan_dead_rows(self._h.value, n))
+        return [dict(rows=flat[2 * s], launches=flat[2 * s + 1]) for s in range(n)]
 
     def backward(self, dwav):
         _, T = self._shape
diff --git a/include/diffmusic_hip.h b/include/diffmusic_hip.h
--- a/include/diffmusic_hip.h
+++ b/include/diffmusic_hip.h
@@ -73,6 +73,9 @@
 int dmx_hifigan_fwd_dead(dmx_model* m, const uint16_t* mel, float* wav, int batch, int frames, int s0, int s1, void* ws,
                          size_t ws_bytes, void* stream);
 int dmx_hifigan_dead_plan(dmx_model* m, int* skipped, int* total, int* lo, int* hi, int n);
+int dmx_hifigan_set_dead_rows(dmx_model* m, int mode);
+int dmx_hifigan_dead_rows(dmx_model* m, int* rows, int* launches, int n);
+int dmx_gemm_rows_plan(int M, int live_M, int N, int K, int mode, int* cfg, int* tiles);
 int dmx_conv_dead_rows(int k, int dil, int pad, int stride, int transposed, int t_in, int t_out, int a, int b, int* lo, int* hi);
 
 size_t dmx_vae_workspace_bytes(dmx_model* m, int batch, int h, int w);
@@ -222,6 +225,7 @@
 int dmx_prof_dominant(double* ms, double* flops, double* bytes);
 
 int dmx_gemm_raw(const void* desc, size_t desc_bytes, void* stream);
+int dmx_gemm_rows_raw(const void* desc, size_t desc_bytes, const int* gap, int cfg, void* stream);
 int dmx_flash_attn_raw(const void* q, const void* k, const void* v, void* o, const float* colbias, int B, int Nq, int Nk, int ldv,
                        int C, int heads, float scale, void* stream);
 int dmx_flash_attn_ld_raw(const void* q, const void* k, const void* v, void* o, const float* colbias, int B, int Nq, int Nk, int ldq,
```

Result: no change. 26.98 steps/s (weak scaling: one step advances a batch of 8 clips on one GPU; value = K / wall x 1 GPU(s)), median of 6 (+0.7%).
